# mycophonic/saprobe-alac

Measured on AMD Instinct MI355X. Metric: Msamples/s decoded (16-bit stereo, 4096-frame packets), higher is better.
Workload: dtype int32; 1 GPU; 65536 packets/GPU x 16-bit 2-ch 4096-frame ALAC, music-like synthetic, device-resident in/out; packets_per_gpu=65536

## Files before the change

saprobe-alac_amd/csrc/alac_gpu.h:

```cpp
#ifndef ALAC_GPU_H
#define ALAC_GPU_H
#include <hip/hip_runtime.h>

#include <algorithm>
#include <cstdio>
#include <cstdlib>
#include <cstring>

#define ALAC_DEV __device__ __forceinline__
#define ALAC_HD __host__ __device__ __forceinline__
#define ALAC_NOINLINE
#define ALAC_MUL24(a, b) __mul24((int)(a), (int)(b))
__device__ __forceinline__ uint32_t alac_sad(uint32_t a, uint32_t b, uint32_t c) {
    uint32_t r;
    asm("v_sad_u32 %0, %1, %2, %3" : "=v"(r) : "v"(a), "v"(b), "v"(c));
    return r;
}
#define ALAC_SAD(a, b, c) alac_sad((uint32_t)(a), (uint32_t)(b), (uint32_t)(c))

__device__ __forceinline__ int32_t alac_sign_med3(int32_t x) {
    int32_t r;
    asm("v_med3_i32 %0, %1, -1, 1" : "=v"(r) : "v"(x));
    return r;
}
#define ALAC_SIGN(x) alac_sign_med3(x)
__device__ __forceinline__ int32_t alac_clamp01_med3(int32_t x) {
    int32_t r;
    asm("v_med3_i32 %0, %1, 0, 1" : "=v"(r) : "v"(x));
    return r;
}
#define ALAC_CLAMP01(x) alac_clamp01_med3(x)
__device__ __forceinline__ uint32_t alac_xad(uint32_t a, uint32_t b, uint32_t c) {
    uint32_t r;
    asm("v_xad_u32 %0, %1, %2, %3" : "=v"(r) : "v"(a), "v"(b), "v"(c));
    return r;
}
#define ALAC_XAD(a, b, c) alac_xad((uint32_t)(a), (uint32_t)(b), (uint32_t)(c))
__device__ __forceinline__ uint32_t alac_not_add(uint32_t a, uint32_t c) {
    uint32_t r;
    asm("v_xad_u32 %0, %1, -1, %2" : "=v"(r) : "v"(a), "v"(c));
    return r;
}
#define ALAC_NOT_ADD(a, c) alac_not_add((uint32_t)(a), (uint32_t)(c))
__device__ __forceinline__ uint32_t alac_bfi(uint32_t m, uint32_t a, uint32_t b) {
    uint32_t r;
    asm("v_bfi_b32 %0, %1, %2, %3" : "=v"(r) : "v"(m), "v"(a), "v"(b));
    return r;
}
#define ALAC_BFI(m, a, b) alac_bfi((uint32_t)(m), (uint32_t)(a), (uint32_t)(b))
__device__ __forceinline__ int32_t alac_mad24(int32_t a, int32_t b, int32_t c) {
    int32_t r;
    asm("v_mad_i32_i24 %0, %1, %2, %3" : "=v"(r) : "v"(a), "v"(b), "v"(c));
    return r;
}
#define ALAC_MAD24(a, b, c) alac_mad24((int32_t)(a), (int32_t)(b), (int32_t)(c))
__device__ __forceinline__ int32_t alac_msub24(int32_t acc, int32_t a, int32_t negc) {
    int32_t r;
    asm("v_mad_i32_i24 %0, %1, %2, %3" : "=v"(r) : "v"(a), "s"(negc), "v"(acc));
    return r;
}
#define ALAC_MSUB24(acc, a, c) alac_msub24((int32_t)(acc), (int32_t)(a), -(int32_t)(c))
#define ALAC_SUBSAT(a, b) __builtin_elementwise_sub_sat((uint32_t)(a), (uint32_t)(b))
__device__ __forceinline__ uint32_t alac_ffbh(uint32_t x) {
    uint32_t r;
    asm("v_ffbh_u32 %0, %1" : "=v"(r) : "v"(x));
    return r;
}
#define ALAC_FFBH(x) alac_ffbh((uint32_t)(x))
__device__ __forceinline__ uint32_t alac_bfe(uint32_t x, uint32_t off, uint32_t width) {
    uint32_t r;
    asm("v_bfe_u32 %0, %1, %2, %3" : "=v"(r) : "v"(x), "v"(off), "v"(width));
    return r;
}
#define ALAC_BFE(x, off, width) alac_bfe((uint32_t)(x), (uint32_t)(off), (uint32_t)(width))
__device__ __forceinline__ int32_t alac_sext_bits(int32_t x, uint32_t bits) {
    int32_t r;
    asm("v_bfe_i32 %0, %1, 0, %2" : "=v"(r) : "v"(x), "v"(bits));
    return r;
}
#define ALAC_SEXT_BITS(x, bits) alac_sext_bits((int32_t)(x), (uint32_t)(bits))
#define ALAC_MULU24(a, b) __umul24((unsigned)(a), (unsigned)(b))
#define ALAC_MULHI(a, b) __umulhi((unsigned)(a), (unsigned)(b))
#define ALAC_ALIGNBIT(hi, lo, sh) __builtin_amdgcn_alignbit((unsigned)(hi), (unsigned)(lo), (unsigned)(sh))
__device__ __forceinline__ int32_t alac_med3_0(int32_t x, int32_t m) {
    int32_t r;
    asm("v_med3_i32 %0, %1, 0, %2" : "=v"(r) : "v"(x), "v"(m));
    return r;
}
#define ALAC_MED3_0(x, m) alac_med3_0((int32_t)(x), (int32_t)(m))
#define ALAC_PACK_LO16(x, y) __builtin_amdgcn_perm((uint32_t)(y), (uint32_t)(x), 0x05040100u)
#define ALAC_PACK_HI16(x, y) __builtin_amdgcn_perm((uint32_t)(y), (uint32_t)(x), 0x07060302u)
__device__ __forceinline__ uint32_t alac_pk_add16(uint32_t a, uint32_t b) {
    uint32_t r;
    asm("v_pk_add_u16 %0, %1, %2" : "=v"(r) : "v"(a), "v"(b));
    return r;
}
#define ALAC_PK_ADD16(a, b) alac_pk_add16((uint32_t)(a), (uint32_t)(b))
__device__ __forceinline__ uint32_t alac_pk_sub16(uint32_t a, uint32_t b) {
    uint32_t r;
    asm("v_pk_sub_u16 %0, %1, %2" : "=v"(r) : "v"(a), "v"(b));
    return r;
}
#define ALAC_PK_SUB16(a, b) alac_pk_sub16((uint32_t)(a), (uint32_t)(b))
#define ALAC_PICK(dst, src) asm volatile("v_mov_b32 %0, %1" : "+v"(dst) : "v"(src))
#define ALAC_OWN_REG(x) asm volatile("" : "+v"(x))
typedef uint32_t alac_u32x4_a4 __attribute__((ext_vector_type(4), aligned(4)));
#define ALAC_LOAD4(q, a, b, c, d)                                                       \
    do {                                                                                \
        const alac_u32x4_a4 v_ = *reinterpret_cast<const alac_u32x4_a4*>(q);            \
        (a) = v_.x;                                                                     \
        (b) = v_.y;                                                                     \
        (c) = v_.z;                                                                     \
        (d) = v_.w;                                                                     \
    } while (0)
typedef int32_t alac_i32x4 __attribute__((ext_vector_type(4)));
#define ALAC_LOAD4_I32(q, a, b, c, d)                                                  \
    do {                                                                               \
        const alac_i32x4 v_ = *reinterpret_cast<const alac_i32x4*>(q);  \
        (a) = v_.x;                                                                    \
        (b) = v_.y;                                                                    \
        (c) = v_.z;                                                                    \
        (d) = v_.w;                                                                    \
    } while (0)
#define ALAC_STORE4(q, a, b, c, d) (*reinterpret_cast<alac_i32x4*>(q) = alac_i32x4{(a), (b), (c), (d)})
#include "alac_wave.h"
#include "alac_regular.h"
#include "alac_duo.h"
#include "alac_split.h"

#define ALAC_PRIO_B_LONG 3
#define ALAC_PRIO_B_MID 2
#define ALAC_PRIO_B_SHORT 1
#define ALAC_PRIO_A 2
#define ALAC_PRIO_C 3

namespace alack {


typedef uint32_t u32x4 __attribute__((ext_vector_type(4)));

constexpr uint32_t kWave = 64;
constexpr uint32_t kTimingSlots = 64;
#ifndef ALAC_LDS_ROWS
#define ALAC_LDS_ROWS 64
#endif
#ifndef ALAC_LDS_RING
#define ALAC_LDS_RING 32
#endif
#ifndef ALAC_LDS_FLUSH
#define ALAC_LDS_FLUSH (ALAC_LDS_ROWS / 2)
#endif
constexpr uint32_t kRing = ALAC_LDS_ROWS;
constexpr uint32_t kFlush = ALAC_LDS_FLUSH;
static_assert(kFlush <= kRing && kRing % 4 == 0 && (kFlush == 16 || kFlush == 32), "the stager flushes 64- or 128-byte pieces of its rows");
constexpr uint32_t kRowStride = kRing + 1;
constexpr uint32_t kFallbackSlots = 64;
constexpr uint32_t kRingDw = ALAC_LDS_RING;
constexpr uint32_t kRingSlots = kRingDw + 2;

constexpr uint32_t kKeys = alac::KEY_IRREGULAR + 2u;
constexpr uint32_t kKeyLegacy = alac::KEY_IRREGULAR;
constexpr uint32_t kKeyScan = alac::KEY_IRREGULAR + 1u;
struct Plan {
    uint32_t count[kKeys];
    uint32_t pkt_start[kKeys];
    uint32_t cursor[kKeys];
    uint32_t nk;
    uint32_t list_key[kKeys];
    uint32_t list_wave0[kKeys];
    uint32_t total_waves;
    uint32_t irr_waves;
    uint32_t wide_waves;
    uint32_t gate[2][512];
    uint32_t balance[2][512];
    uint32_t queue[2];
};

static __shared__ uint32_t s_rows[kWave * kRowStride];
static __shared__ unsigned long long s_optr[kWave];
static __shared__ __attribute__((aligned(16))) uint32_t s_ring[kRingSlots * kWave];
constexpr uint32_t kQ = alac::DUO_CHUNK;
static __shared__ int32_t s_rq[2 * kQ * kWave];

__host__ __device__ inline size_t u_tile_cells(uint32_t frame_length) { return ((size_t)frame_length + 1u) * kWave; }

struct GpuWave {
    static constexpr bool kResMem = false;
    static constexpr uint32_t kRingDw = alack::kRingDw;
    int32_t* u_tile;
    int32_t* g_tile;
    uint8_t* my_out;
    uint32_t lane, wcnt, flushed;
    uint32_t ppw;

    ALAC_DEV bool any(bool p) const { return __ballot(p) != 0ull; }
    ALAC_DEV uint32_t max_u32(uint32_t v) const {
#pragma unroll
        for (int o = 32; o > 0; o >>= 1) {
            const uint32_t t = (uint32_t)__shfl_xor((int)v, o, 64);
            v = t > v ? t : v;
        }
        return (uint32_t)__builtin_amdgcn_readfirstlane((int)v);
    }
    static constexpr bool kRingPow2 = (kRing & (kRing - 1u)) == 0u;
    uint32_t wpos, fpos;
    ALAC_DEV static uint32_t umin_(uint32_t a, uint32_t b) { return a < b ? a : b; }
    ALAC_DEV static uint32_t st_wrap(uint32_t x) { return kRingPow2 ? (x & (kRing - 1u)) : umin_(x, x - kRing); }
    ALAC_DEV uint32_t st_pos() const { return kRingPow2 ? (wcnt & (kRing - 1u)) : wpos; }
    ALAC_DEV void st_adv(uint32_t n) {
        wcnt += n;
        if (!kRingPow2) wpos = st_wrap(wpos + n);
    }
    ALAC_DEV void st_begin(uint8_t* out) {
        my_out = out;
        s_optr[lane] = (unsigned long long)reinterpret_cast<uintptr_t>(out);
        wcnt = flushed = 0;
        wpos = fpos = 0;
    }
    ALAC_DEV void st_push(uint32_t v) {
        s_rows[lane * kRowStride + st_pos()] = v;
        st_adv(1u);
    }
    ALAC_DEV void st_push_if(uint32_t v, bool on) {
        s_rows[lane * kRowStride + st_pos()] = v;
        st_adv(on ? 1u : 0u);
    }
    ALAC_DEV uint32_t st_group_base(uint32_t un) const { return lane * kRowStride + (kRingPow2 ? (wcnt & (kRing - un)) : wpos); }
    ALAC_DEV void st_put(uint32_t base, uint32_t j, uint32_t v, uint32_t) { s_rows[base + j] = v; }
    ALAC_DEV void st_advance(uint32_t n) { st_adv(n); }
    ALAC_DEV void st_push6_n(uint32_t d0, uint32_t d1, uint32_t d2, uint32_t d3, uint32_t d4, uint32_t d5, uint32_t count) {
        const uint32_t pos = st_pos();
        uint32_t* row = s_rows + lane * kRowStride;
        if (pos <= kRing - 6u) {
            uint32_t* r = row + pos;
            r[0] = d0;
            r[1] = d1;
            r[2] = d2;
            r[3] = d3;
            r[4] = d4;
            r[5] = d5;
        } else {
            row[pos] = d0;
            row[st_wrap(pos + 1u)] = d1;
            row[st_wrap(pos + 2u)] = d2;
            row[st_wrap(pos + 3u)] = d3;
            row[st_wrap(pos + 4u)] = d4;
            row[st_wrap(pos + 5u)] = d5;
        }
        st_adv(count);
    }
    ALAC_DEV void st_tail(uint64_t acc, uint32_t nbytes) {
        for (uint32_t b = 0; b < nbytes; ++b) my_out[(size_t)wcnt * 4u + b] = (uint8_t)(acc >> (8u * b));
    }
    ALAC_DEV void st_step() {
        constexpr uint32_t LPP = kFlush / 4u;
        constexpr uint32_t PPI = kWave / LPP;
        const bool full = (wcnt - flushed) >= kFlush;
        const unsigned long long mask = __ballot(full);
        if (mask == 0ull) return;
        __builtin_amdgcn_wave_barrier();
        const int first = __ffsll((long long)mask) - 1;
        const uint32_t fl = (uint32_t)__shfl((int)flushed, first, 64);
        const uint32_t col0 = kRingPow2 ? (fl & (kRing - 1u)) : (uint32_t)__shfl((int)fpos, first, 64);
        const uint32_t piece = lane & (LPP - 1u);
        const uint32_t groups = (ppw + PPI - 1u) / PPI;
        const uint32_t col = st_wrap(col0 + piece * 4u);
        for (uint32_t k = 0; k < groups; ++k) {
            const uint32_t q = PPI * k + lane / LPP;
            if ((mask >> q) & 1ull) {
                const uint32_t* r = s_rows + q * kRowStride + col;
                const uint4 v = make_uint4(r[0], r[1], r[2], r[3]);
                uint8_t* dst = reinterpret_cast<uint8_t*>((uintptr_t)s_optr[q]) + ((size_t)fl + piece * 4u) * 4u;
                *reinterpret_cast<__attribute__((address_space(1))) u32x4*>((uintptr_t)dst) = u32x4{v.x, v.y, v.z, v.w};
            }
        }
        __builtin_amdgcn_wave_barrier();
        if (full) {
            flushed += kFlush;
            if (!kRingPow2) fpos = st_wrap(fpos + kFlush);
        }
    }
    ALAC_DEV uint32_t st_finish() {
        uint32_t c = kRingPow2 ? 0u : fpos;
        for (uint32_t w = flushed; w < wcnt; ++w) {
            *reinterpret_cast<uint32_t*>(my_out + (size_t)w * 4u) = s_rows[lane * kRowStride + (kRingPow2 ? (w & (kRing - 1u)) : c)];
            if (!kRingPow2) c = st_wrap(c + 1u);
        }
        flushed = wcnt;
        if (!kRingPow2) fpos = wpos;
        return wcnt;
    }
    ALAC_DEV void ring_write4(uint32_t slot, uint32_t a, uint32_t b, uint32_t c, uint32_t d) {
        uint32_t* q = &s_ring[slot * kWave + lane];
        q[0] = a;
        q[kWave] = b;
        q[2 * kWave] = c;
        q[3 * kWave] = d;
    }
    ALAC_DEV uint32_t ring_read(uint32_t slot) const { return s_ring[slot * kWave + lane]; }
    ALAC_DEV void ring_read2(uint32_t slot, uint32_t& a, uint32_t& b) const {
        const uint32_t* q = &s_ring[slot * kWave + lane];
        a = q[0];
        b = q[kWave];
    }
    ALAC_DEV void ring_read2_at(uint32_t byte_off, uint32_t& a, uint32_t& b) const {
        const uint32_t* q = reinterpret_cast<const uint32_t*>(reinterpret_cast<const char*>(&s_ring[lane]) + byte_off * kWave);
        a = q[0];
        b = q[kWave];
    }
    ALAC_DEV void ring_write1(uint32_t slot, uint32_t v) { s_ring[slot * kWave + lane] = v; }
    ALAC_DEV void rq_write(uint32_t buf, uint32_t j, int32_t v) { s_rq[(buf * kQ + j) * kWave + lane] = v; }
    ALAC_DEV int32_t rq_read(uint32_t buf, uint32_t j) const { return s_rq[(buf * kQ + j) * kWave + lane]; }
    ALAC_DEV uint32_t pair_hi(uint32_t x) const { return (uint32_t)__builtin_amdgcn_mov_dpp((int)x, 0xF5, 0xf, 0xf, true); }
    ALAC_DEV int32_t pair_sum(int32_t x) const { return x + __builtin_amdgcn_mov_dpp(x, 0xB1, 0xf, 0xf, true); }
    ALAC_DEV uint32_t pair_from_below(uint32_t x, uint32_t fresh, uint32_t q0m) const {
        return ALAC_BFI(q0m, fresh, (uint32_t)__builtin_amdgcn_mov_dpp((int)x, 0xA0, 0xf, 0xf, true));
    }
    template <int L>
    ALAC_DEV uint32_t quad_from(uint32_t x) const {
        return (uint32_t)__builtin_amdgcn_mov_dpp((int)x, L * 0x55, 0xf, 0xf, true);
    }
    template <int D>
    ALAC_DEV uint32_t quad_up(uint32_t x) const {
        constexpr int c = D == 1 ? 0xF9 : D == 2 ? 0xFE : 0xFF;
        return (uint32_t)__builtin_amdgcn_mov_dpp((int)x, c, 0xf, 0xf, true);
    }
    ALAC_DEV int32_t quad_sum(int32_t x) const {
        const int32_t y = x + __builtin_amdgcn_mov_dpp(x, 0xB1, 0xf, 0xf, true);
        return y + __builtin_amdgcn_mov_dpp(y, 0x4E, 0xf, 0xf, true);
    }
    ALAC_DEV uint32_t quad_from_below(uint32_t x, uint32_t fresh, uint32_t q0m) const {
        return ALAC_BFI(q0m, fresh, (uint32_t)__builtin_amdgcn_mov_dpp((int)x, 0x90, 0xf, 0xf, true));
    }
    ALAC_DEV void duo_sync() { asm volatile("s_waitcnt lgkmcnt(0)\n\ts_barrier" ::: "memory"); }
    ALAC_DEV void duo_sync_mem() {
        __threadfence_block();
        __syncthreads();
    }
    ALAC_DEV int32_t* u_row(uint32_t i) const { return u_tile + ((size_t)i * kWave + (ppw < kWave ? (lane < ppw ? lane : ppw) : lane)); }
    ALAC_DEV int32_t* g_slot(uint32_t k) const { return g_tile + (size_t)k * ppw; }
};

struct GpuWaveMem : GpuWave {
    static constexpr bool kResMem = true;
    const int32_t* res;
    uint32_t it, chunk0;
    ALAC_DEV int32_t rq_read(uint32_t, uint32_t j) const { return res[chunk0 + j]; }
    ALAC_DEV void rq_write(uint32_t, uint32_t, int32_t) {}
    ALAC_DEV void duo_sync() {
        ++it;
        chunk0 = (it - 1u) * kQ;
    }
    ALAC_DEV void duo_sync_mem() {}
};

__device__ __forceinline__ uint32_t avail_of(uint64_t blob_bytes, uint64_t off) {
    const uint64_t left = blob_bytes - off;
    return left > 0xffffffffull ? 0xffffffffu : (uint32_t)left;
}

__global__ void alac_classify(alac::DevCfg cfg, const uint8_t* __restrict__ blob, uint64_t blob_bytes, const uint64_t* __restrict__ offsets,
                              const uint32_t* __restrict__ sizes, uint32_t n, uint16_t* __restrict__ keys, uint32_t* __restrict__ sizes_ws,
                              uint32_t* __restrict__ frames_out, int32_t* __restrict__ status, Plan* plan);
__global__ void alac_plan(Plan* plan, uint32_t ppw);
__global__ void alac_cu_census(uint32_t* __restrict__ seen, uint32_t* __restrict__ arrived, uint32_t expect);
__global__ void alac_scatter(const uint16_t* __restrict__ keys, uint32_t n, Plan* plan, uint32_t* __restrict__ perm);
__global__ void alac_task_classify(alac::DevCfg cfg, const alac::ChanDesc* __restrict__ cd, const alac::PktDesc* __restrict__ pd,
                                   const uint16_t* __restrict__ pkt_keys, uint32_t n_slots, uint16_t* __restrict__ keys, Plan* plan);
__global__ void alac_scan(alac::DevCfg cfg, const uint8_t* __restrict__ blob, uint64_t blob_bytes, const uint64_t* __restrict__ offsets,
                          const uint32_t* __restrict__ sizes, const uint32_t* __restrict__ perm, const Plan* __restrict__ plan,
                          uint8_t* __restrict__ out, uint64_t out_stride, uint32_t* __restrict__ frames_out,
                          int32_t* __restrict__ status, int32_t* __restrict__ scratch_u, int32_t* __restrict__ scratch_g,
                          uint32_t ppw, alac::ChanDesc* __restrict__ cd, alac::PktDesc* __restrict__ pd, int32_t* __restrict__ rows,
                          uint64_t row_stride);
__global__ void alac_legacy(alac::DevCfg cfg, const uint8_t* __restrict__ blob, uint64_t blob_bytes, const uint64_t* __restrict__ offsets,
                            const uint32_t* __restrict__ sizes, const uint32_t* __restrict__ perm, const Plan* __restrict__ plan,
                            const alac::PktDesc* __restrict__ pd, uint8_t* __restrict__ out, uint64_t out_stride,
                            uint32_t* __restrict__ frames_out, int32_t* __restrict__ status, int32_t* __restrict__ scratch_u,
                            int32_t* __restrict__ scratch_g, uint32_t ppw);
constexpr uint32_t kModeFit4 = 4u, kModeFit5 = 5u, kModeGated = 6u;
constexpr __host__ __device__ __forceinline__ uint32_t decode_mode(uint32_t items, uint32_t n_cu, uint32_t cap, uint32_t force, bool mono,
                                                                  bool fit5) {
    if (force == kModeFit4 || (force == kModeFit5 && fit5)) return force;
    if (items <= 4u * n_cu) return kModeFit4;
    if (items <= 5u * n_cu) return (cap >= 5u && !mono) ? kModeGated : fit5 ? kModeFit5 : kModeFit4;
    if (items <= 6u * n_cu && cap >= 6u) return kModeGated;
    return (2u * items <= 15u * n_cu || !fit5) ? kModeFit4 : kModeFit5;
}
constexpr __host__ __device__ __forceinline__ uint32_t pair_quota(uint32_t items, uint32_t n_cu, uint32_t cap) {
    const uint32_t need = (items + n_cu - 1u) / n_cu;
    return need < 5u ? 5u : need < cap ? need : cap;
}
constexpr bool mode_is_fit4_without_the_others(uint32_t n_cu) {
    for (uint32_t items = 0u; items <= 40u * n_cu; items += (items < 8u * n_cu ? 1u : n_cu / 2u + 1u))
        if (decode_mode(items, n_cu, 0u, 0u, false, false) != kModeFit4 || decode_mode(items, n_cu, 0u, 5u, true, false) != kModeFit4) return false;
    return true;
}
constexpr bool mode_is_fit4_within_four(uint32_t n_cu) {
    for (uint32_t cap = 0u; cap <= 8u; ++cap)
        for (uint32_t items = 0u; items <= 4u * n_cu; ++items)
            if (decode_mode(items, n_cu, cap, 0u, false, true) != kModeFit4 || decode_mode(items, n_cu, cap, 0u, true, true) != kModeFit4) return false;
    return true;
}
static_assert(mode_is_fit4_without_the_others(1u) && mode_is_fit4_without_the_others(64u) && mode_is_fit4_without_the_others(256u) &&
                  mode_is_fit4_within_four(1u) && mode_is_fit4_within_four(7u) && mode_is_fit4_within_four(64u) &&
                  mode_is_fit4_within_four(256u) && mode_is_fit4_within_four(304u),
              "decode_mode would leave batches of up to 4 x CUs wave slots to a launch that is not made for them");
constexpr uint32_t kQuadLdsFit4 = 34816u;

struct PairArgs {
    alac::DevCfg cfg;
    const uint8_t* blob;
    uint64_t blob_bytes;
    const uint64_t* offsets;
    const uint32_t* sizes;
    const uint32_t* perm;
    Plan* plan;
    uint8_t* out;
    uint64_t out_stride;
    uint32_t* frames_out;
    int32_t* status;
    int32_t* scratch_u;
    const uint32_t* cu_number;
    uint32_t* claims;
    uint32_t ppw;
    uint32_t n_cu;
    uint32_t cap;
    uint32_t lanes_min;
    uint32_t fit;
    uint32_t fit_force;
    uint32_t fit5;
};
#define ALAC_DECLARE_DECODE(NAME) __global__ void NAME(PairArgs);
ALAC_DECLARE_DECODE(alac_decode_16q) ALAC_DECLARE_DECODE(alac_decode_16g) ALAC_DECLARE_DECODE(alac_decode_24q) ALAC_DECLARE_DECODE(alac_decode_32q)
ALAC_DECLARE_DECODE(alac_decode_w24) ALAC_DECLARE_DECODE(alac_decode_w32)
#undef ALAC_DECLARE_DECODE
__global__ void alac_chan_predict(alac::DevCfg cfg, const uint8_t* __restrict__ blob, uint64_t blob_bytes, const uint64_t* __restrict__ offsets,
                                  const uint32_t* __restrict__ sizes, const uint32_t* __restrict__ perm, const Plan* __restrict__ plan,
                                  const alac::ChanDesc* __restrict__ cd, int32_t* __restrict__ rows, uint64_t row_stride, uint32_t ppw);
__global__ void alac_interleave(alac::DevCfg cfg, const uint8_t* __restrict__ blob, uint64_t blob_bytes, const uint64_t* __restrict__ offsets,
                                const uint32_t* __restrict__ sizes, const uint32_t* __restrict__ perm, const Plan* __restrict__ plan,
                                const alac::ChanDesc* __restrict__ cd, const alac::PktDesc* __restrict__ pd, const int32_t* __restrict__ rows,
                                uint64_t row_stride, uint8_t* __restrict__ out, uint64_t out_stride, uint32_t blocks_per_pkt);
__global__ void alac_interleave4(alac::DevCfg cfg, const uint8_t* __restrict__ blob, uint64_t blob_bytes, const uint64_t* __restrict__ offsets,
                                const uint32_t* __restrict__ sizes, const uint32_t* __restrict__ perm, const Plan* __restrict__ plan,
                                const alac::ChanDesc* __restrict__ cd, const alac::PktDesc* __restrict__ pd, const int32_t* __restrict__ rows,
                                uint64_t row_stride, uint8_t* __restrict__ out, uint64_t out_stride, uint32_t blocks_per_pkt);

}
#endif
```

saprobe-alac_amd/csrc/alacgpu.hip:

```cpp
#include "alac_gpu.h"
#include "alac_host.h"
#include "alac_waveform.h"
#include "alac_clips.h"

using namespace alack;

namespace {
thread_local char g_err[512] = "";
}

void alack::set_err(const char* fmt, ...) {
    va_list ap;
    va_start(ap, fmt);
    vsnprintf(g_err, sizeof(g_err), fmt, ap);
    va_end(ap);
}

namespace {

class CopyPool {
public:
    explicit CopyPool(unsigned threads) {
        for (unsigned t = 0; t < threads; ++t) workers_.emplace_back([this] { run(); });
    }
    ~CopyPool() {
        {
            std::lock_guard<std::mutex> g(m_);
            stop_ = true;
        }
        cv_.notify_all();
        for (auto& w : workers_) w.join();
    }
    void parallel_for(size_t tasks, const std::function<void(size_t)>& fn) {
        if (tasks == 0) return;
        if (workers_.empty() || tasks == 1) {
            for (size_t k = 0; k < tasks; ++k) fn(k);
            return;
        }
        {
            std::lock_guard<std::mutex> g(m_);
            fn_ = &fn;
            tasks_ = tasks;
            next_ = 0;
            left_ = tasks;
            ++gen_;
        }
        cv_.notify_all();
        work();
        std::unique_lock<std::mutex> l(m_);
        done_.wait(l, [this] { return left_ == 0; });
        fn_ = nullptr;
    }

private:
    void work() {
        for (;;) {
            size_t k;
            const std::function<void(size_t)>* fn;
            {
                std::lock_guard<std::mutex> g(m_);
                if (!fn_ || next_ >= tasks_) return;
                k = next_++;
                fn = fn_;
            }
            (*fn)(k);
            std::lock_guard<std::mutex> g(m_);
            if (--left_ == 0) done_.notify_all();
        }
    }
    void run() {
        uint64_t seen = 0;
        for (;;) {
            {
                std::unique_lock<std::mutex> l(m_);
                cv_.wait(l, [&] { return stop_ || gen_ != seen; });
                if (stop_) return;
                seen = gen_;
            }
            work();
        }
    }
    std::vector<std::thread> workers_;
    std::mutex m_;
    std::condition_variable cv_, done_;
    const std::function<void(size_t)>* fn_ = nullptr;
    size_t tasks_ = 0, next_ = 0, left_ = 0;
    uint64_t gen_ = 0;
    bool stop_ = false;
};

void copy_pieces(CopyPool* pool, size_t pieces, const std::function<void(size_t)>& fn) {
    if (pool) pool->parallel_for(pieces, fn);
    else for (size_t k = 0; k < pieces; k++) fn(k);
}

constexpr int kSlots = 3;

struct Slot {
    DevBuf d_in;
    DevBuf d_out;
    HostBuf h_in, h_out;
    hipEvent_t ev_in = nullptr, ev_k = nullptr, ev_out = nullptr;
    size_t first = 0, n = 0;
    bool busy = false;
    bool bad = false;
};

struct PairKernel {
    void (*fn)(PairArgs);
    const char* name;
};
struct Kernels {
    bool lean;
    bool one_or_two;
    PairKernel quad;
    PairKernel gated;
    PairKernel wide;
    decltype(&alac_interleave) interleave;
    uint32_t interleave_lds;
    const char* irregular;
};
#define ALAC_PAIR_KERNEL(k) PairKernel{k, #k}
Kernels choose_kernels(const alac::DevCfg& c) {
    Kernels k{};
    k.lean = alac::lean_config(c);
    k.one_or_two = c.num_channels <= 2;
    k.quad = c.bit_depth == 16 ? ALAC_PAIR_KERNEL(alac_decode_16q) : c.bit_depth == 32 ? ALAC_PAIR_KERNEL(alac_decode_32q) : ALAC_PAIR_KERNEL(alac_decode_24q);
    k.gated = c.bit_depth == 16 ? ALAC_PAIR_KERNEL(alac_decode_16g) : PairKernel{nullptr, ""};
    k.wide = c.bit_depth == 32 ? ALAC_PAIR_KERNEL(alac_decode_w32) : c.bit_depth == 24 ? ALAC_PAIR_KERNEL(alac_decode_w24) : PairKernel{nullptr, ""};
    const bool four_frames = c.num_channels > 2 && (c.num_channels * c.bps) % 4u == 0u;
    k.interleave = four_frames ? alac_interleave4 : alac_interleave;
    k.interleave_lds = (four_frames ? 128u : 32u) * kWave;
    k.irregular = !k.lean        ? "alac_scan (whole-packet decoder)"
                  : k.one_or_two ? "alac_scan + alac_interleave (+ alac_legacy)"
                  : four_frames  ? "alac_scan + alac_chan_predict + alac_interleave4 (+ alac_legacy)"
                                 : "alac_scan + alac_chan_predict + alac_interleave (+ alac_legacy)";
    return k;
}
#undef ALAC_PAIR_KERNEL

}

struct alacgpu_decoder {
    alacgpu_config cfg;
    alac::DevCfg dev_cfg;
    Kernels kernels;
    int device;
    size_t frame_bytes;
    hipStream_t stream;
    hipStream_t s_in, s_out;
    hipStream_t s_side;
    hipEvent_t ev_fork, ev_join;
    hipEvent_t ev_start[kTimingSlots], ev_stop[kTimingSlots];
    uint64_t launches;
    DevBuf scratch_u, scratch_g, plan, cls, perm, sizes_ws;
    DevBuf cd, pd, plan2, keys2, perm2, rows;
    Slot slots[kSlots];
    CopyPool* pool;
    uint32_t n_cu;
    DevBuf cu_number;
    size_t chunk_bytes;
    uint32_t lanes_min;
    int side;
    std::thread* ahead;
    int ahead_rc;
    char ahead_err[512];
    size_t last_n;
    uint32_t last_ppw, last_cap, last_fit5;
    uint32_t fit_force;
    DevBuf wave_ws;
    hipEvent_t ev_w0, ev_w1;
    bool wave_timed;
    hipEvent_t ev_c0, ev_c1;
    bool clips_timed;
};

namespace {

size_t plan_claims_offset() { return (sizeof(Plan) + 255u) & ~(size_t)255u; }
size_t plan_bytes(size_t waves) { return plan_claims_offset() + waves * 4 * sizeof(uint32_t); }

struct KernelAttr {
    uint32_t pairs_per_cu, static_lds;
};
KernelAttr kernel_attr(void (*kernel)(PairArgs)) {
    static std::mutex mu;
    static std::vector<std::pair<const void*, KernelAttr>> cache;
    std::lock_guard<std::mutex> g(mu);
    for (const auto& e : cache)
        if (e.first == (const void*)kernel) return e.second;
    int v = 0;
    hipFuncAttributes at;
    KernelAttr a{4u, kQuadLdsFit4};
    if (hipOccupancyMaxActiveBlocksPerMultiprocessor(&v, kernel, (int)(2 * kWave), 0) == hipSuccess && v > 0) a.pairs_per_cu = (uint32_t)v;
    else (void)hipGetLastError();
    if (hipFuncGetAttributes(&at, (const void*)kernel) == hipSuccess) a.static_lds = (uint32_t)at.sharedSizeBytes;
    else (void)hipGetLastError();
    cache.emplace_back((const void*)kernel, a);
    return a;
}

int cu_numbers(alacgpu_decoder* dec) {
    int rc;
    if ((rc = dec->cu_number.ensure(513 * sizeof(uint32_t)))) return rc;
    HIP_TRY(hipMemsetAsync(dec->cu_number.p, 0, 513 * sizeof(uint32_t), dec->stream));
    hipLaunchKernelGGL(alac_cu_census, dim3(2 * dec->n_cu), dim3(kWave), 0, dec->stream, (uint32_t*)dec->cu_number.p,
                       (uint32_t*)dec->cu_number.p + 512, 2 * dec->n_cu);
    HIP_TRY(hipGetLastError());
    uint32_t seen[512];
    HIP_TRY(hipMemcpyAsync(seen, dec->cu_number.p, sizeof(seen), hipMemcpyDeviceToHost, dec->stream));
    HIP_TRY(hipStreamSynchronize(dec->stream));
    uint32_t per_xcd[8] = {0}, xcds = 0, total = 0;
    for (uint32_t i = 0; i < 512; i++)
        if (seen[i]) {
            per_xcd[i >> 6]++;
            total++;
        }
    for (uint32_t x = 0; x < 8; x++) xcds += per_xcd[x] ? 1u : 0u;
    if (xcds == 0) xcds = 1;
    uint32_t next[8] = {0}, order[8] = {0}, k = 0;
    for (uint32_t x = 0; x < 8; x++)
        if (per_xcd[x]) order[x] = k++;
    for (uint32_t i = 0; i < 512; i++)
        if (seen[i]) {
            const uint32_t x = i >> 6;
            seen[i] = 1u + next[x]++ * xcds + order[x];
        }
    if (total > dec->n_cu) dec->n_cu = total;
    HIP_TRY(hipMemcpyAsync(dec->cu_number.p, seen, sizeof(seen), hipMemcpyHostToDevice, dec->stream));
    HIP_TRY(hipStreamSynchronize(dec->stream));
    return ALACGPU_E_OK;
}

size_t max_waves(uint32_t bit_depth, size_t n, uint32_t ppw) {
    const size_t keys = (bit_depth >= 24 ? 2 : 1) * 18 * 18 + 8;
    return (n + ppw - 1) / ppw + std::min<size_t>(n, keys);
}
size_t max_waves(const alacgpu_decoder* dec, size_t n, uint32_t ppw) { return max_waves(dec->cfg.bit_depth, n, ppw); }

uint32_t pick_ppw(size_t n) {
    if (const char* e = getenv("ALACGPU_PPW")) {
        const int v = atoi(e);
        if (v >= 1 && v <= 64) return (uint32_t)v;
    }
    uint32_t ppw = kWave;
    while (ppw > 1 && n / ppw < 256) ppw >>= 1;
    return ppw;
}

size_t row_stride_of(uint32_t frame_length) { return ((size_t)frame_length + 3u) & ~(size_t)3u; }

int reserve_workspace(alacgpu_decoder* dec, size_t n, uint32_t ppw) {
    const size_t waves = max_waves(dec, n, ppw);
    int rc;
    if ((rc = dec->scratch_u.ensure(waves * u_tile_cells(dec->cfg.frame_length) * sizeof(int32_t)))) return rc;
    if ((rc = dec->scratch_g.ensure(waves * kFallbackSlots * ppw * sizeof(int32_t)))) return rc;
    if ((rc = dec->plan.ensure(plan_bytes(waves)))) return rc;
    if ((rc = dec->cls.ensure((n ? n : 1) * sizeof(uint16_t)))) return rc;
    if ((rc = dec->perm.ensure((n ? n : 1) * sizeof(uint32_t)))) return rc;
    if ((rc = dec->sizes_ws.ensure((n ? n : 1) * sizeof(uint32_t)))) return rc;
    const size_t ns = (n ? n : 1) * 8;
    if ((rc = dec->cd.ensure(ns * sizeof(alac::ChanDesc)))) return rc;
    if ((rc = dec->pd.ensure((n ? n : 1) * sizeof(alac::PktDesc)))) return rc;
    if (dec->cfg.num_channels > 2) {
        if ((rc = dec->plan2.ensure(sizeof(Plan)))) return rc;
        if ((rc = dec->keys2.ensure(ns * sizeof(uint16_t)))) return rc;
        if ((rc = dec->perm2.ensure(ns * sizeof(uint32_t)))) return rc;
        if ((rc = dec->rows.ensure((n ? n : 1) * dec->cfg.num_channels * row_stride_of(dec->cfg.frame_length) * sizeof(int32_t))))
            return rc;
    }
    return ALACGPU_E_OK;
}

struct Launch {
    alacgpu_decoder* dec;
    alac::DevCfg c;
    const uint8_t* d_blob;
    uint64_t blob_bytes;
    const uint64_t* d_offsets;
    size_t n;
    uint8_t* d_out;
    size_t out_stride;
    uint32_t* d_frames;
    int32_t* d_status;
    uint32_t ppw;
    size_t waves;
    hipStream_t irr;
    bool forked;
    uint32_t scan_grid;
    Plan* plan() const { return (Plan*)dec->plan.p; }
    const uint32_t* sz() const { return (const uint32_t*)dec->sizes_ws.p; }
};

struct SideFork {
    alacgpu_decoder* dec;
    bool open = false;
    int fork() {
        HIP_TRY(hipEventRecord(dec->ev_fork, dec->stream));
        HIP_TRY(hipStreamWaitEvent(dec->s_side, dec->ev_fork, 0));
        open = true;
        return ALACGPU_E_OK;
    }
    int join() {
        HIP_TRY(hipEventRecord(dec->ev_join, dec->s_side));
        HIP_TRY(hipStreamWaitEvent(dec->stream, dec->ev_join, 0));
        open = false;
        return ALACGPU_E_OK;
    }
    ~SideFork() {
        if (open) (void)hipStreamSynchronize(dec->s_side);
    }
};

int sort_pass(const Launch& L, const uint32_t* d_sizes) {
    alacgpu_decoder* dec = L.dec;
    const uint32_t nb = (uint32_t)((L.n + 255) / 256);
    HIP_TRY(hipMemsetAsync(L.plan(), 0, plan_bytes(L.waves), dec->stream));
    hipLaunchKernelGGL(alac_classify, dim3(nb), dim3(256), 0, dec->stream, L.c, L.d_blob, L.blob_bytes, L.d_offsets, d_sizes,
                       (uint32_t)L.n, (uint16_t*)dec->cls.p, (uint32_t*)dec->sizes_ws.p, L.d_frames, L.d_status, L.plan());
    hipLaunchKernelGGL(alac_plan, dim3(1), dim3(kWave), 0, dec->stream, L.plan(), L.ppw);
    hipLaunchKernelGGL(alac_scatter, dim3(nb), dim3(256), 0, dec->stream, (const uint16_t*)dec->cls.p, (uint32_t)L.n, L.plan(),
                       (uint32_t*)dec->perm.p);
    return ALACGPU_E_OK;
}

void scan(const Launch& L) {
    alacgpu_decoder* dec = L.dec;
    hipLaunchKernelGGL(alac_scan, dim3(L.scan_grid), dim3(kWave), 0, L.irr, L.c, L.d_blob, L.blob_bytes,
                       L.d_offsets, L.sz(), (const uint32_t*)dec->perm.p, (const Plan*)L.plan(), L.d_out, (uint64_t)L.out_stride, L.d_frames,
                       L.d_status, (int32_t*)dec->scratch_u.p, (int32_t*)dec->scratch_g.p, L.ppw, (alac::ChanDesc*)dec->cd.p,
                       (alac::PktDesc*)dec->pd.p, dec->cfg.num_channels > 2 ? (int32_t*)dec->rows.p : (int32_t*)nullptr,
                       (uint64_t)row_stride_of(dec->cfg.frame_length));
}

void narrow_launch(const Launch& L, const PairArgs& a, uint32_t slots, uint32_t mode) {
    alacgpu_decoder* dec = L.dec;
    const Kernels& k = dec->kernels;
    if (mode == kModeGated) {
        if (a.cap) hipLaunchKernelGGL(k.gated.fn, dim3(std::min<uint32_t>(a.cap * dec->n_cu, slots)), dim3(2 * kWave), 0, dec->stream, a);
        return;
    }
    if (mode == kModeFit5 && !a.fit5) return;
    const uint32_t stat = kernel_attr(k.quad.fn).static_lds;
    PairArgs q = a;
    q.fit = mode;
    hipLaunchKernelGGL(k.quad.fn, dim3(slots), dim3(4 * kWave), (mode == kModeFit4 && stat < kQuadLdsFit4) ? kQuadLdsFit4 - stat : 0u,
                       dec->stream, q);
}

void regular_packets(const Launch& L) {
    alacgpu_decoder* dec = L.dec;
    const Kernels& k = dec->kernels;
    const size_t n = L.n;
    const uint32_t ppw = L.ppw;
    PairArgs a{L.c, L.d_blob, (uint64_t)L.blob_bytes, L.d_offsets, L.sz(), (const uint32_t*)dec->perm.p, L.plan(), L.d_out, (uint64_t)L.out_stride,
               L.d_frames, L.d_status, (int32_t*)dec->scratch_u.p, (const uint32_t*)dec->cu_number.p,
               (uint32_t*)((uint8_t*)L.plan() + plan_claims_offset()), ppw, dec->n_cu, 0u, dec->lanes_min, 4u, dec->fit_force, 0u};
    const uint32_t slots = (uint32_t)L.waves;
    const uint32_t n_cu = dec->n_cu;
    const bool beyond4 = (n + ppw - 1) / ppw > (size_t)4 * n_cu || dec->fit_force == kModeFit5;
    const bool has_twin = k.gated.fn && beyond4 && dec->fit_force == 0u;
    {
        const uint32_t stat = kernel_attr(k.quad.fn).static_lds;
        a.fit5 = (beyond4 && (size_t)((stat + 1279u) / 1280u) * 1280u * 5u <= 163840u) ? 1u : 0u;
    }
    if (has_twin) a.cap = kernel_attr(k.gated.fn).pairs_per_cu;
    if (a.cap <= 4u) a.cap = 0u;
    dec->last_cap = a.cap;
    dec->last_fit5 = a.fit5;
    const uint32_t guess = decode_mode((uint32_t)((n + ppw - 1) / ppw), n_cu, a.cap, dec->fit_force, dec->cfg.num_channels == 1, a.fit5 != 0u);
    narrow_launch(L, a, slots, guess);
    if (k.wide.fn) hipLaunchKernelGGL(k.wide.fn, dim3(slots), dim3(2 * kWave), 0, dec->stream, a);
    for (uint32_t mode : {kModeFit4, kModeFit5, kModeGated})
        if (mode != guess) narrow_launch(L, a, slots, mode);
}

int split_pipeline(const Launch& L) {
    alacgpu_decoder* dec = L.dec;
    Plan* plan2 = (Plan*)dec->plan2.p;
    const size_t n_slots = L.n * 8;
    const uint32_t nb2 = (uint32_t)((n_slots + 255) / 256);
    const uint32_t ppw2 = pick_ppw(L.n * dec->cfg.num_channels);
    HIP_TRY(hipMemsetAsync(plan2, 0, sizeof(Plan), dec->stream));
    hipLaunchKernelGGL(alac_task_classify, dim3(nb2), dim3(256), 0, dec->stream, L.c, (const alac::ChanDesc*)dec->cd.p,
                       (const alac::PktDesc*)dec->pd.p, (const uint16_t*)dec->cls.p, (uint32_t)n_slots,
                       (uint16_t*)dec->keys2.p, plan2);
    hipLaunchKernelGGL(alac_plan, dim3(1), dim3(kWave), 0, dec->stream, plan2, ppw2);
    hipLaunchKernelGGL(alac_scatter, dim3(nb2), dim3(256), 0, dec->stream, (const uint16_t*)dec->keys2.p,
                       (uint32_t)n_slots, plan2, (uint32_t*)dec->perm2.p);
    hipLaunchKernelGGL(alac_chan_predict, dim3((uint32_t)max_waves(16u, n_slots, ppw2)), dim3(kWave), 0, dec->stream, L.c,
                       L.d_blob, L.blob_bytes, L.d_offsets, L.sz(), (const uint32_t*)dec->perm2.p, (const Plan*)plan2,
                       (const alac::ChanDesc*)dec->cd.p, (int32_t*)dec->rows.p, (uint64_t)row_stride_of(dec->cfg.frame_length), ppw2);
    return ALACGPU_E_OK;
}

void irregular_pcm(const Launch& L) {
    alacgpu_decoder* dec = L.dec;
    const Kernels& k = dec->kernels;
    const uint64_t rs = row_stride_of(dec->cfg.frame_length);
    const uint32_t bpp = (dec->cfg.frame_length + kWave - 1u) / kWave;
    const uint32_t ib = (uint32_t)std::min<uint64_t>((uint64_t)L.n * ((bpp + 7u) / 8u), L.forked ? (uint64_t)4 * dec->n_cu : (uint64_t)32768u);
    hipLaunchKernelGGL(k.interleave, dim3(ib), dim3(kWave), k.interleave_lds, L.irr, L.c, L.d_blob, L.blob_bytes, L.d_offsets, L.sz(),
                       (const uint32_t*)dec->perm.p, (const Plan*)L.plan(), (const alac::ChanDesc*)dec->cd.p,
                       (const alac::PktDesc*)dec->pd.p, (const int32_t*)dec->rows.p, rs, L.d_out, (uint64_t)L.out_stride, bpp);
    hipLaunchKernelGGL(alac_legacy, dim3(L.scan_grid), dim3(kWave), 0, L.irr, L.c, L.d_blob, L.blob_bytes,
                       L.d_offsets, L.sz(), (const uint32_t*)dec->perm.p, (const Plan*)L.plan(), (const alac::PktDesc*)dec->pd.p, L.d_out,
                       (uint64_t)L.out_stride, L.d_frames, L.d_status, (int32_t*)dec->scratch_u.p, (int32_t*)dec->scratch_g.p, L.ppw);
}

int launch(alacgpu_decoder* dec, const uint8_t* d_blob, uint64_t blob_bytes, const uint64_t* d_offsets,
           const uint32_t* d_sizes, size_t n, uint8_t* d_out, size_t out_stride, uint32_t* d_frames, int32_t* d_status) {
    if (n == 0) return ALACGPU_E_OK;
    if (n > 0x7fffffffu) {
        set_err("batch too large");
        return ALACGPU_E_ARG;
    }
    const uint32_t ppw = pick_ppw(n);
    int rc = reserve_workspace(dec, n, ppw);
    if (rc) return rc;
    dec->last_n = n;
    dec->last_ppw = ppw;
    dec->last_cap = dec->last_fit5 = 0;
    const Kernels& k = dec->kernels;
    Launch L{dec, dec->dev_cfg, d_blob, blob_bytes, d_offsets, n, d_out, out_stride, d_frames, d_status, ppw, max_waves(dec, n, ppw),
             dec->stream, false, 0u};
    L.c.aligned16 = (out_stride % 16 == 0 && (reinterpret_cast<uintptr_t>(d_out) % 16) == 0) ? 1u : 0u;
    const uint32_t slot = (uint32_t)(dec->launches % kTimingSlots);
    HIP_TRY(hipEventRecord(dec->ev_start[slot], dec->stream));
    if ((rc = sort_pass(L, d_sizes))) return rc;
    L.forked = k.one_or_two && k.lean &&
               (dec->side >= 2 || (dec->side == 1 && (n + ppw - 1) / ppw <= (size_t)6 * dec->n_cu));
    L.scan_grid = (uint32_t)std::min<size_t>(L.waves, (size_t)(L.forked ? 2u : 6u) * dec->n_cu);
    SideFork side{dec};
    if (L.forked) {
        if ((rc = side.fork())) return rc;
        L.irr = dec->s_side;
    }
    if (!L.forked) scan(L);
    if (k.one_or_two && k.lean) regular_packets(L);
    if (L.forked) scan(L);
    HIP_TRY(hipGetLastError());
    if (k.lean) {
        if (!k.one_or_two && (rc = split_pipeline(L))) return rc;
        irregular_pcm(L);
        HIP_TRY(hipGetLastError());
    }
    if (L.forked && (rc = side.join())) return rc;
    HIP_TRY(hipEventRecord(dec->ev_stop[slot], dec->stream));
    dec->launches++;
    return ALACGPU_E_OK;
}

}

namespace {
std::mutex g_pool_mu;
std::vector<alacgpu_decoder*> g_pool;
std::vector<std::pair<void*, size_t>> g_host_pool;
std::vector<std::pair<void*, size_t>> g_host_sizes;
constexpr size_t kPoolPerDevice = 4;
constexpr size_t kPoolKeepDevice = (size_t)2048 << 20;
constexpr size_t kPoolKeepPinned = (size_t)64 << 20;
constexpr size_t kHostPoolBlock = (size_t)64 << 20, kHostPoolBytes = (size_t)192 << 20, kHostPoolCount = 8;
template <class Buf>
void keep_at_most(std::vector<Buf*> bufs, size_t limit) {
    for (;;) {
        size_t total = 0;
        Buf* big = nullptr;
        for (Buf* b : bufs) {
            total += b->cap;
            if (b->cap && (!big || b->cap > big->cap)) big = b;
        }
        if (total <= limit || !big) return;
        big->release();
    }
}

std::vector<DevBuf*> device_buffers(alacgpu_decoder* d) {
    std::vector<DevBuf*> v = {&d->scratch_u, &d->scratch_g, &d->plan, &d->cls, &d->perm, &d->sizes_ws, &d->cd, &d->pd,
                              &d->plan2, &d->keys2, &d->perm2, &d->rows, &d->wave_ws};
    for (Slot& s : d->slots) v.insert(v.end(), {&s.d_in, &s.d_out});
    return v;
}
std::vector<HostBuf*> pinned_buffers(alacgpu_decoder* d) {
    std::vector<HostBuf*> v;
    for (Slot& s : d->slots) v.insert(v.end(), {&s.h_in, &s.h_out});
    return v;
}
std::vector<hipStream_t*> streams_of(alacgpu_decoder* d) { return {&d->stream, &d->s_in, &d->s_out, &d->s_side}; }
struct EventRef {
    hipEvent_t* ev;
    unsigned flags;
};
std::vector<EventRef> events_of(alacgpu_decoder* d) {
    std::vector<EventRef> v = {{&d->ev_fork, hipEventDisableTiming}, {&d->ev_join, hipEventDisableTiming},
                               {&d->ev_w0, hipEventDefault}, {&d->ev_w1, hipEventDefault},
                               {&d->ev_c0, hipEventDefault}, {&d->ev_c1, hipEventDefault}};
    for (uint32_t i = 0; i < kTimingSlots; i++) v.insert(v.end(), {{&d->ev_start[i], hipEventDefault}, {&d->ev_stop[i], hipEventDefault}});
    for (Slot& s : d->slots)
        v.insert(v.end(), {{&s.ev_in, hipEventDisableTiming}, {&s.ev_k, hipEventDisableTiming}, {&s.ev_out, hipEventDisableTiming}});
    return v;
}

bool synchronize_all(alacgpu_decoder* d) {
    bool ok = true;
    for (hipStream_t* s : streams_of(d))
        if (*s && hipStreamSynchronize(*s) != hipSuccess) ok = false;
    return ok;
}

void really_destroy(alacgpu_decoder* d) {
    (void)hipSetDevice(d->device);
    (void)synchronize_all(d);
    delete d->pool;
    d->cu_number.release();
    for (DevBuf* b : device_buffers(d)) b->release();
    for (HostBuf* b : pinned_buffers(d)) b->release();
    for (const EventRef& e : events_of(d))
        if (*e.ev) (void)hipEventDestroy(*e.ev);
    for (hipStream_t* s : streams_of(d))
        if (*s) (void)hipStreamDestroy(*s);
    delete d;
}

void configure(alacgpu_decoder* d, const alacgpu_config* cfg) {
    const uint32_t bps = alacwf::bytes_per_sample(cfg->bit_depth);
    d->cfg = *cfg;
    d->frame_bytes = (size_t)cfg->frame_length * cfg->num_channels * (size_t)bps;
    d->dev_cfg = alac::DevCfg{cfg->frame_length, cfg->bit_depth, cfg->num_channels, cfg->pb, cfg->mb, cfg->kb, bps, 0u};
    d->kernels = choose_kernels(d->dev_cfg);
    d->launches = 0;
    d->ahead = nullptr;
    d->ahead_rc = ALACGPU_E_OK;
    d->ahead_err[0] = 0;
    d->last_n = 0;
    d->last_ppw = d->last_cap = d->last_fit5 = 0;
    d->wave_timed = false;
    d->clips_timed = false;
    d->lanes_min = 4;
    d->fit_force = 0;
    if (const char* e = getenv("ALACGPU_FIT")) d->fit_force = (uint32_t)atoi(e);
    if (const char* e = getenv("ALACGPU_LANES_MIN")) d->lanes_min = (uint32_t)std::max(1, atoi(e));
    d->side = 2;
    if (const char* e = getenv("ALACGPU_SIDE")) d->side = atoi(e);
    d->chunk_bytes = (size_t)192 << 20;
    if (const char* e = getenv("ALACGPU_CHUNK_MB")) {
        const long v = atol(e);
        if (v >= 1 && v <= 65536) d->chunk_bytes = (size_t)v << 20;
    }
}
}

static int settle_ahead(alacgpu_decoder* d);

static int check_decode_args(const alacgpu_decoder* d, const void* blob, size_t blob_bytes, const void* offsets, size_t n, const void* out,
                             size_t out_stride, const void* frames, const void* status) {
    if (!d || (n && (!offsets || !out || !frames || !status)) || (blob_bytes && !blob)) {
        set_err("null argument");
        return ALACGPU_E_ARG;
    }
    if (out_stride < d->frame_bytes) {
        set_err("out_stride %zu < frame bytes %zu", out_stride, d->frame_bytes);
        return ALACGPU_E_ARG;
    }
    return ALACGPU_E_OK;
}

extern "C" {

int alacgpu_create(const alacgpu_config* cfg, int device, alacgpu_decoder** out) {
    if (!cfg || !out) {
        set_err("null argument");
        return ALACGPU_E_ARG;
    }
    *out = nullptr;
    if (int rc = check_config(cfg)) return rc;
    HIP_TRY(hipSetDevice(device));
    {
        std::lock_guard<std::mutex> g(g_pool_mu);
        for (size_t i = 0; i < g_pool.size(); i++)
            if (g_pool[i]->device == device) {
                alacgpu_decoder* d = g_pool[i];
                g_pool.erase(g_pool.begin() + (long)i);
                configure(d, cfg);
                *out = d;
                return ALACGPU_E_OK;
            }
    }
    alacgpu_decoder* d = new (std::nothrow) alacgpu_decoder();
    if (!d) {
        set_err("out of memory");
        return ALACGPU_E_ARG;
    }
    d->device = device;
    configure(d, cfg);
    {
        int cus = 0;
        if (hipDeviceGetAttribute(&cus, hipDeviceAttributeMultiprocessorCount, device) != hipSuccess) cus = 0;
        d->n_cu = cus > 0 ? (uint32_t)cus : 256u;
    }
    hipError_t e = hipSuccess;
    for (hipStream_t* st : streams_of(d))
        if (e == hipSuccess) e = hipStreamCreateWithFlags(st, hipStreamNonBlocking);
    for (const EventRef& ev : events_of(d))
        if (e == hipSuccess) e = hipEventCreateWithFlags(ev.ev, ev.flags);
    if (e != hipSuccess) {
        set_err("stream/event creation failed: %s", hipGetErrorString(e));
        really_destroy(d);
        return ALACGPU_E_HIP;
    }
    if (int rc = cu_numbers(d)) {
        really_destroy(d);
        return rc;
    }
    *out = d;
    return ALACGPU_E_OK;
}

void alacgpu_destroy(alacgpu_decoder* d) {
    if (!d) return;
    (void)settle_ahead(d);
    (void)hipSetDevice(d->device);
    if (synchronize_all(d)) {
        for (int k = 0; k < kSlots; k++) d->slots[k].busy = false;
        keep_at_most(device_buffers(d), kPoolKeepDevice);
        keep_at_most(pinned_buffers(d), kPoolKeepPinned);
        std::lock_guard<std::mutex> g(g_pool_mu);
        size_t same = 0;
        for (alacgpu_decoder* p : g_pool) same += p->device == d->device ? 1u : 0u;
        if (same < kPoolPerDevice) {
            g_pool.push_back(d);
            return;
        }
    }
    really_destroy(d);
}

void alacgpu_trim(void) {
    std::vector<alacgpu_decoder*> all;
    std::vector<std::pair<void*, size_t>> host;
    {
        std::lock_guard<std::mutex> g(g_pool_mu);
        all.swap(g_pool);
        host.swap(g_host_pool);
    }
    for (alacgpu_decoder* d : all) really_destroy(d);
    for (auto& h : host) (void)hipHostFree(h.first);
}

void* alacgpu_host_alloc(size_t bytes) {
    if (bytes == 0) bytes = 1;
    {
        std::lock_guard<std::mutex> g(g_pool_mu);
        size_t best = SIZE_MAX;
        for (size_t i = 0; i < g_host_pool.size(); i++)
            if (g_host_pool[i].second >= bytes && g_host_pool[i].second <= 2 * bytes + (1u << 20) &&
                (best == SIZE_MAX || g_host_pool[i].second < g_host_pool[best].second))
                best = i;
        if (best != SIZE_MAX) {
            void* p = g_host_pool[best].first;
            g_host_sizes.emplace_back(p, g_host_pool[best].second);
            g_host_pool.erase(g_host_pool.begin() + (long)best);
            return p;
        }
    }
    void* p = nullptr;
    if (hipHostMalloc(&p, bytes, hipHostMallocDefault) != hipSuccess) {
        (void)hipGetLastError();
        set_err("hipHostMalloc(%zu) failed", bytes);
        return nullptr;
    }
    std::lock_guard<std::mutex> g(g_pool_mu);
    g_host_sizes.emplace_back(p, bytes);
    return p;
}

void alacgpu_host_free(void* p) {
    if (!p) return;
    size_t bytes = 0;
    std::vector<void*> evict;
    {
        std::lock_guard<std::mutex> g(g_pool_mu);
        for (size_t i = 0; i < g_host_sizes.size(); i++)
            if (g_host_sizes[i].first == p) {
                bytes = g_host_sizes[i].second;
                g_host_sizes.erase(g_host_sizes.begin() + (long)i);
                break;
            }
        if (bytes && bytes <= kHostPoolBlock) {
            g_host_pool.emplace_back(p, bytes);
            p = nullptr;
            size_t total = 0;
            for (const auto& h : g_host_pool) total += h.second;
            while (g_host_pool.size() > kHostPoolCount || total > kHostPoolBytes) {
                evict.push_back(g_host_pool.front().first);
                total -= g_host_pool.front().second;
                g_host_pool.erase(g_host_pool.begin());
            }
        }
    }
    for (void* q : evict) (void)hipHostFree(q);
    if (p) (void)hipHostFree(p);
}

int alacgpu_get_format(const alacgpu_decoder* d, alacgpu_format* fmt) {
    if (!d || !fmt) return ALACGPU_E_ARG;
    fmt->sample_rate = (int32_t)d->cfg.sample_rate;
    fmt->bit_depth = d->cfg.bit_depth;
    fmt->channels = d->cfg.num_channels;
    return ALACGPU_E_OK;
}

size_t alacgpu_frame_bytes(const alacgpu_decoder* d) { return d ? d->frame_bytes : 0; }

int alacgpu_reserve(alacgpu_decoder* d, size_t n) {
    if (!d) return ALACGPU_E_ARG;
    HIP_TRY(hipSetDevice(d->device));
    if (int rc = d->wave_ws.ensure(alack::wave_scratch_bytes(n))) return rc;
    return reserve_workspace(d, n, pick_ppw(n));
}

static int settle_ahead(alacgpu_decoder* d) {
    if (!d->ahead) return ALACGPU_E_OK;
    d->ahead->join();
    delete d->ahead;
    d->ahead = nullptr;
    if (d->ahead_rc != ALACGPU_E_OK) set_err("%s", d->ahead_err);
    return d->ahead_rc;
}

int alacgpu_decode_batch_start(alacgpu_decoder* d, const uint8_t* blob, size_t blob_bytes, const uint64_t* offsets, size_t n,
                               uint8_t* out, size_t out_stride, uint32_t* frames_out, int32_t* status) {
    if (!d) return ALACGPU_E_ARG;
    if (d->ahead) {
        set_err("a decode started with alacgpu_decode_batch_start is still in flight: alacgpu_decode_batch_wait first");
        return ALACGPU_E_ARG;
    }
    d->ahead_rc = ALACGPU_E_OK;
    d->ahead = new (std::nothrow) std::thread([=] {
        d->ahead_rc = alacgpu_decode_batch(d, blob, blob_bytes, offsets, n, out, out_stride, frames_out, status);
        if (d->ahead_rc != ALACGPU_E_OK) snprintf(d->ahead_err, sizeof(d->ahead_err), "%s", alacgpu_last_error());
    });
    if (!d->ahead) {
        set_err("out of memory");
        return ALACGPU_E_ARG;
    }
    return ALACGPU_E_OK;
}

int alacgpu_decode_batch_wait(alacgpu_decoder* d) {
    if (!d) return ALACGPU_E_ARG;
    return settle_ahead(d);
}

int alacgpu_decode_batch_device(alacgpu_decoder* d, const uint8_t* d_blob, size_t blob_bytes, const uint64_t* d_offsets,
                                const uint32_t* d_sizes, size_t n, uint8_t* d_out, size_t out_stride,
                                uint32_t* d_frames, int32_t* d_status, int sync) {
    int rc = check_decode_args(d, d_blob, blob_bytes, d_offsets, n, d_out, out_stride, d_frames, d_status);
    if (rc) return rc;
    HIP_TRY(hipSetDevice(d->device));
    rc = launch(d, d_blob, (uint64_t)blob_bytes, d_offsets, d_sizes, n, d_out, out_stride, d_frames, d_status);
    if (rc) return rc;
    if (sync) HIP_TRY(hipStreamSynchronize(d->stream));
    return ALACGPU_E_OK;
}

int alacgpu_decode_batch(alacgpu_decoder* d, const uint8_t* blob, size_t blob_bytes, const uint64_t* offsets, size_t n,
                         uint8_t* out, size_t out_stride, uint32_t* frames_out, int32_t* status) {
    if (int rc = check_decode_args(d, blob, blob_bytes, offsets, n, out, out_stride, frames_out, status)) return rc;
    if (n == 0) return ALACGPU_E_OK;
    auto valid = [&](size_t i) {
        const uint64_t lo = offsets[i], hi = offsets[i + 1];
        return lo <= hi && hi <= (uint64_t)blob_bytes && hi - lo <= 0x0fffffffull;
    };
    HIP_TRY(hipSetDevice(d->device));
    const size_t fb = d->frame_bytes;
    const size_t d_stride = (fb + 15u) & ~(size_t)15u;
    const bool out_pinned = is_pinned(out) && is_pinned(frames_out) && is_pinned(status);
    const bool in_pinned = blob_bytes == 0 || is_pinned(blob);
    if (!d->pool && !(out_pinned && in_pinned)) {
        unsigned t = std::thread::hardware_concurrency();
        t = t > 16 ? 8 : (t > 2 ? t / 2 : 1);
        if (const char* e = getenv("ALACGPU_COPY_THREADS")) t = (unsigned)std::max(1, atoi(e));
        d->pool = new (std::nothrow) CopyPool(t - 1);
    }

    auto finish = [&](Slot& s) -> int {
        HIP_TRY(hipEventSynchronize(s.ev_out));
        if (!out_pinned) {
            const uint8_t* h = (const uint8_t*)s.h_out.p;
            const uint8_t* hm = h + s.n * d_stride;
            memcpy(frames_out + s.first, hm, s.n * sizeof(uint32_t));
            memcpy(status + s.first, hm + s.n * sizeof(uint32_t), s.n * sizeof(int32_t));
            const size_t pieces = std::min<size_t>(s.n, 64);
            auto body = [&](size_t k) {
                const size_t lo = s.n * k / pieces, hi = s.n * (k + 1) / pieces;
                if (out_stride == fb && d_stride == fb) {
                    memcpy(out + (s.first + lo) * out_stride, h + lo * d_stride, (hi - lo) * fb);
                } else {
                    for (size_t i = lo; i < hi; i++) memcpy(out + (s.first + i) * out_stride, h + i * d_stride, fb);
                }
            };
            copy_pieces(d->pool, pieces, body);
        }
        if (s.bad)
            for (size_t i = s.first; i < s.first + s.n; i++)
                if (!valid(i)) {
                    status[i] = ALACGPU_ERR_RANGE;
                    frames_out[i] = 0;
                }
        {
            const size_t bpf = fb / d->cfg.frame_length;
            for (size_t i = s.first; i < s.first + s.n; i++) {
                const size_t have = std::min<size_t>(frames_out[i], d->cfg.frame_length) * bpf;
                if (have < fb) memset(out + i * out_stride + have, 0, fb - have);
            }
        }
        s.busy = false;
        return ALACGPU_E_OK;
    };
    auto submit = [&](Slot& s, size_t first, size_t cnt, uint64_t lo, uint64_t hi) -> int {
        int rc;
        s.first = first;
        s.n = cnt;
        s.bad = false;
        const size_t in_bytes = (size_t)(hi - lo);
        const size_t meta = (cnt + 1) * sizeof(uint64_t) + cnt * sizeof(uint32_t);
        const size_t meta_pad = (meta + 255u) & ~(size_t)255u;
        if ((rc = s.d_in.ensure(meta_pad + in_bytes + 16))) return rc;
        if ((rc = s.d_out.ensure(cnt * d_stride + cnt * 8 + 16))) return rc;
        if ((rc = s.h_in.ensure(in_pinned ? meta_pad : meta_pad + in_bytes))) return rc;
        if (!out_pinned && (rc = s.h_out.ensure(cnt * d_stride + cnt * 8))) return rc;
        uint64_t* h_off = (uint64_t*)s.h_in.p;
        uint32_t* h_sz = (uint32_t*)(h_off + cnt + 1);
        for (size_t i = 0; i < cnt; i++) {
            const bool ok = valid(first + i);
            h_off[i] = ok ? offsets[first + i] - lo : 0u;
            h_sz[i] = ok ? (uint32_t)(offsets[first + i + 1] - offsets[first + i]) : 0u;
            s.bad = s.bad || !ok;
        }
        h_off[cnt] = in_bytes;
        uint8_t* d_in = (uint8_t*)s.d_in.p;
        if (in_pinned) {
            HIP_TRY(hipMemcpyAsync(d_in, h_off, meta, hipMemcpyHostToDevice, d->s_in));
            if (in_bytes) HIP_TRY(hipMemcpyAsync(d_in + meta_pad, blob + lo, in_bytes, hipMemcpyHostToDevice, d->s_in));
        } else {
            uint8_t* hb = (uint8_t*)s.h_in.p + meta_pad;
            const size_t pieces = std::max<size_t>(1, std::min<size_t>(64, in_bytes >> 20));
            auto body = [&](size_t k) {
                const size_t a = in_bytes * k / pieces, b = in_bytes * (k + 1) / pieces;
                memcpy(hb + a, blob + lo + a, b - a);
            };
            copy_pieces(d->pool, pieces, body);
            HIP_TRY(hipMemcpyAsync(d_in, s.h_in.p, meta_pad + in_bytes, hipMemcpyHostToDevice, d->s_in));
        }
        HIP_TRY(hipEventRecord(s.ev_in, d->s_in));
        HIP_TRY(hipStreamWaitEvent(d->stream, s.ev_in, 0));
        uint8_t* d_pcm = (uint8_t*)s.d_out.p;
        uint32_t* d_fr = (uint32_t*)(d_pcm + cnt * d_stride);
        int32_t* d_st = (int32_t*)(d_fr + cnt);
        if ((rc = launch(d, d_in + meta_pad, in_bytes, (const uint64_t*)d_in, (const uint32_t*)(d_in + (cnt + 1) * sizeof(uint64_t)), cnt,
                         d_pcm, d_stride, d_fr, d_st)))
            return rc;
        HIP_TRY(hipEventRecord(s.ev_k, d->stream));
        HIP_TRY(hipStreamWaitEvent(d->s_out, s.ev_k, 0));
        if (out_pinned) {
            HIP_TRY(hipMemcpy2DAsync(out + first * out_stride, out_stride, d_pcm, d_stride, fb, cnt, hipMemcpyDeviceToHost, d->s_out));
            HIP_TRY(hipMemcpyAsync(frames_out + first, d_fr, cnt * sizeof(uint32_t), hipMemcpyDeviceToHost, d->s_out));
            HIP_TRY(hipMemcpyAsync(status + first, d_st, cnt * sizeof(int32_t), hipMemcpyDeviceToHost, d->s_out));
        } else {
            HIP_TRY(hipMemcpyAsync(s.h_out.p, d_pcm, cnt * d_stride + cnt * 8, hipMemcpyDeviceToHost, d->s_out));
        }
        HIP_TRY(hipEventRecord(s.ev_out, d->s_out));
        s.busy = true;
        return ALACGPU_E_OK;
    };

    size_t first = 0;
    int turn = 0;
    int rc = ALACGPU_E_OK;
    while (first < n && rc == ALACGPU_E_OK) {
        size_t cnt = 0;
        uint64_t lo = ~0ull, hi = 0;
        while (first + cnt < n) {
            uint64_t nlo = lo, nhi = hi;
            if (valid(first + cnt)) {
                nlo = std::min(lo, offsets[first + cnt]);
                nhi = std::max(hi, offsets[first + cnt + 1]);
            }
            const uint64_t bytes = (nhi > nlo ? nhi - nlo : 0) + (uint64_t)(cnt + 1) * fb;
            if (cnt != 0 && bytes > d->chunk_bytes) break;
            lo = nlo;
            hi = nhi;
            cnt++;
        }
        if (hi < lo) lo = hi = 0;
        Slot& s = d->slots[turn];
        turn = (turn + 1) % kSlots;
        if (s.busy && (rc = finish(s))) break;
        rc = submit(s, first, cnt, lo, hi);
        first += cnt;
    }
    if (rc != ALACGPU_E_OK) {
        (void)hipStreamSynchronize(d->s_in);
        (void)hipStreamSynchronize(d->stream);
        (void)hipStreamSynchronize(d->s_side);
        (void)hipStreamSynchronize(d->s_out);
        for (int k = 0; k < kSlots; k++) d->slots[k].busy = false;
        return rc;
    }
    for (int k = 0; k < kSlots; k++) {
        Slot& s = d->slots[(turn + k) % kSlots];
        if (!s.busy) continue;
        const int r2 = finish(s);
        if (rc == ALACGPU_E_OK) rc = r2;
        s.busy = false;
    }
    return rc;
}

int alacgpu_decode_packet(alacgpu_decoder* d, const uint8_t* packet, size_t packet_len, uint8_t* out, size_t out_cap,
                          size_t* out_len, int32_t* status_out) {
    if (!d || (!packet && packet_len) || !out || !out_len) {
        set_err("null argument");
        return ALACGPU_E_ARG;
    }
    if (out_cap < d->frame_bytes) {
        set_err("output capacity %zu < frame bytes %zu", out_cap, d->frame_bytes);
        return ALACGPU_E_ARG;
    }
    *out_len = 0;
    const uint64_t offs[2] = {0, packet_len};
    const uint8_t dummy = 0;
    uint32_t frames = 0;
    int32_t st = 0;
    int rc = alacgpu_decode_batch(d, packet_len ? packet : &dummy, packet_len, offs, 1, out, d->frame_bytes, &frames, &st);
    if (rc) return rc;
    if (status_out) *status_out = st;
    if (st != 0) {
        set_err("decode failed: status 0x%x", st);
        return ALACGPU_E_DECODE;
    }
    *out_len = (size_t)frames * d->cfg.num_channels * (size_t)d->dev_cfg.bps;
    return ALACGPU_E_OK;
}

int alacgpu_timing_reset(alacgpu_decoder* d) {
    if (!d) return ALACGPU_E_ARG;
    d->launches = 0;
    return ALACGPU_E_OK;
}

int alacgpu_kernel_times(alacgpu_decoder* d, float* ms, size_t max_n, size_t* n_out) {
    if (!d || !ms || !n_out) return ALACGPU_E_ARG;
    HIP_TRY(hipSetDevice(d->device));
    HIP_TRY(hipStreamSynchronize(d->stream));
    size_t avail = (size_t)std::min<uint64_t>(d->launches, kTimingSlots);
    size_t n = std::min(avail, max_n);
    for (size_t i = 0; i < n; i++) {
        const uint32_t slot = (uint32_t)((d->launches - n + i) % kTimingSlots);
        HIP_TRY(hipEventElapsedTime(&ms[i], d->ev_start[slot], d->ev_stop[slot]));
    }
    *n_out = n;
    return ALACGPU_E_OK;
}

int alacgpu_pair_placement(alacgpu_decoder* d, uint32_t* tags, size_t max_n, size_t* n_out) {
    if (!d || !tags || !n_out) return ALACGPU_E_ARG;
    HIP_TRY(hipSetDevice(d->device));
    HIP_TRY(hipStreamSynchronize(d->stream));
    *n_out = 0;
    if (!d->plan.p) return ALACGPU_E_OK;
    Plan head;
    HIP_TRY(hipMemcpy(&head, d->plan.p, sizeof(Plan), hipMemcpyDeviceToHost));
    const size_t n = std::min<size_t>(head.total_waves, max_n / 4);
    if (plan_bytes(n) > d->plan.cap) return ALACGPU_E_ARG;
    if (n) HIP_TRY(hipMemcpy(tags, (const uint8_t*)d->plan.p + plan_claims_offset(), n * 4 * sizeof(uint32_t), hipMemcpyDeviceToHost));
    *n_out = n;
    return ALACGPU_E_OK;
}

int alacgpu_last_dispatch(alacgpu_decoder* d, alacgpu_dispatch* out) {
    if (!d || !out) return ALACGPU_E_ARG;
    HIP_TRY(hipSetDevice(d->device));
    HIP_TRY(hipStreamSynchronize(d->stream));
    memset(out, 0, sizeof(*out));
    if (!d->plan.p || d->last_n == 0) return ALACGPU_E_OK;
    Plan head;
    HIP_TRY(hipMemcpy(&head, d->plan.p, sizeof(Plan), hipMemcpyDeviceToHost));
    out->packets_per_slot = d->last_ppw;
    out->slots = head.total_waves;
    out->irregular_slots = head.irr_waves;
    out->wide_slots = head.wide_waves;
    out->narrow_slots = head.total_waves - head.irr_waves - head.wide_waves;
    out->keys = head.nk;
    const Kernels& k = d->kernels;
    const bool lean = k.one_or_two && k.lean;
    const char* narrow = "";
    if (lean && out->narrow_slots) {
        const uint32_t mode = decode_mode(out->narrow_slots, d->n_cu, d->last_cap, d->fit_force, d->cfg.num_channels == 1, d->last_fit5 != 0u);
        narrow = mode == kModeGated ? k.gated.name : k.quad.name;
        out->gated = mode == kModeGated ? 1u : 0u;
        out->workgroups_per_cu = mode == kModeGated ? pair_quota(out->narrow_slots, d->n_cu, d->last_cap) : mode;
        if (!out->gated && out->narrow_slots <= d->n_cu + d->n_cu / 8u && d->lanes_min <= 16u) out->lanes_per_packet = d->last_ppw <= 32u ? 4u : 2u;
    }
    snprintf(out->narrow_kernel, sizeof(out->narrow_kernel), "%s", narrow);
    snprintf(out->wide_kernel, sizeof(out->wide_kernel), "%s", (lean && out->wide_slots) ? k.wide.name : "");
    snprintf(out->irregular_kernels, sizeof(out->irregular_kernels), "%s", out->irregular_slots ? k.irregular : "");
    return ALACGPU_E_OK;
}

int alacgpu_last_kernel_ms(alacgpu_decoder* d, float* ms) {
    size_t got = 0;
    int rc = alacgpu_kernel_times(d, ms, 1, &got);
    if (rc) return rc;
    if (got == 0) {
        set_err("no kernel has been launched on this handle since the last timing reset");
        return ALACGPU_E_ARG;
    }
    return ALACGPU_E_OK;
}

int alacgpu_waveform_device(alacgpu_decoder* d, const uint8_t* d_pcm, size_t pcm_stride, const uint32_t* d_frames,
                            const int32_t* d_status, size_t n, int layout, int type, void* d_wave, size_t channel_stride,
                            size_t packet_stride, uint64_t* d_starts, int sync) {
    if (!d || (n && (!d_pcm || !d_frames || !d_wave))) {
        set_err("null argument");
        return ALACGPU_E_ARG;
    }
    if ((layout != ALACGPU_WAVE_STREAM && layout != ALACGPU_WAVE_PACKETS) || (type != ALACGPU_WAVE_FLOAT && type != ALACGPU_WAVE_INT)) {
        set_err("unknown waveform layout %d or type %d", layout, type);
        return ALACGPU_E_ARG;
    }
    if (n > 0x7fffffffu) {
        set_err("batch too large");
        return ALACGPU_E_ARG;
    }
    const uint64_t fl = d->cfg.frame_length, ch = d->cfg.num_channels;
    if (n) {
        if (pcm_stride < d->frame_bytes) {
            set_err("pcm_stride %zu < frame bytes %zu", pcm_stride, d->frame_bytes);
            return ALACGPU_E_ARG;
        }
        if (reinterpret_cast<uintptr_t>(d_wave) % 4) {
            set_err("d_wave is not aligned to its 4-byte elements");
            return ALACGPU_E_ARG;
        }
        if (layout == ALACGPU_WAVE_STREAM ? channel_stride < (uint64_t)n * fl
                                          : (channel_stride < fl || packet_stride / ch < channel_stride)) {
            set_err("channel_stride %zu / packet_stride %zu too small for %zu packets of %u frames", channel_stride, packet_stride, n,
                    d->cfg.frame_length);
            return ALACGPU_E_ARG;
        }
    }
    HIP_TRY(hipSetDevice(d->device));
    if (n && (layout == ALACGPU_WAVE_STREAM || d_starts)) {
        if (int rc = d->wave_ws.ensure(alack::wave_scratch_bytes(n))) return rc;
    }
    alacwf::Params p = alacwf::make_params(d->cfg.frame_length, d->cfg.bit_depth, d->cfg.num_channels, (uint32_t)layout, (uint32_t)type);
    p.pcm = d_pcm;
    p.pcm_stride = pcm_stride;
    p.frames = d_frames;
    p.status = d_status;
    p.wave = (uint8_t*)d_wave;
    p.channel_stride = channel_stride;
    p.packet_stride = packet_stride;
    p.n = n;
    HIP_TRY(hipEventRecord(d->ev_w0, d->stream));
    HIP_TRY(alack::wave_launch(d->stream, p, d_starts, d->wave_ws.p));
    HIP_TRY(hipEventRecord(d->ev_w1, d->stream));
    d->wave_timed = true;
    if (sync) HIP_TRY(hipStreamSynchronize(d->stream));
    return ALACGPU_E_OK;
}

int alacgpu_waveform_last_ms(alacgpu_decoder* d, float* ms) {
    if (!d || !ms || !d->wave_timed) {
        set_err(!d || !ms ? "null argument" : "no waveform pass on this handle yet");
        return ALACGPU_E_ARG;
    }
    HIP_TRY(hipSetDevice(d->device));
    HIP_TRY(hipEventSynchronize(d->ev_w1));
    HIP_TRY(hipEventElapsedTime(ms, d->ev_w0, d->ev_w1));
    return ALACGPU_E_OK;
}

int alacgpu_clips_device(alacgpu_decoder* d, const uint8_t* d_pcm, size_t pcm_stride, const uint32_t* d_frames,
                         const int32_t* d_status, size_t n, const uint64_t* d_begin, const uint64_t* d_limit, size_t n_clips,
                         uint32_t clip_frames, int type, void* d_clips, size_t channel_stride, size_t clip_stride,
                         uint32_t* d_valid, int32_t* d_clip_status, int sync) {
    if (!d || (n_clips && (!d_pcm || !d_frames || !d_begin || !d_limit || !d_clips))) {
        set_err("null argument");
        return ALACGPU_E_ARG;
    }
    if (type != ALACGPU_WAVE_FLOAT && type != ALACGPU_WAVE_INT) {
        set_err("unknown waveform type %d", type);
        return ALACGPU_E_ARG;
    }
    if (n > 0x7fffffffu || n_clips > 0x7fffffffu) {
        set_err("batch too large");
        return ALACGPU_E_ARG;
    }
    if (n_clips == 0) return ALACGPU_E_OK;
    const uint64_t ch = d->cfg.num_channels;
    if (clip_frames == 0) {
        set_err("clip_frames is 0");
        return ALACGPU_E_ARG;
    }
    if (n && (pcm_stride < d->frame_bytes || pcm_stride > SIZE_MAX / n)) {
        set_err("pcm_stride %zu < frame bytes %zu, or the slots overflow", pcm_stride, d->frame_bytes);
        return ALACGPU_E_ARG;
    }
    if (reinterpret_cast<uintptr_t>(d_clips) % 4) {
        set_err("d_clips is not aligned to its 4-byte elements");
        return ALACGPU_E_ARG;
    }
    if (channel_stride < clip_frames || clip_stride / ch < channel_stride || clip_stride > (SIZE_MAX / 8) / n_clips) {
        set_err("channel_stride %zu / clip_stride %zu too small for clips of %u frames, or the clips overflow", channel_stride, clip_stride,
                clip_frames);
        return ALACGPU_E_ARG;
    }
    HIP_TRY(hipSetDevice(d->device));
    alacclip::Params p = alacclip::make_params(d->cfg.frame_length, d->cfg.bit_depth, d->cfg.num_channels, (uint32_t)type, clip_frames);
    p.pcm = d_pcm;
    p.pcm_stride = pcm_stride;
    p.frames = d_frames;
    p.status = d_status;
    p.n = n;
    p.begin = d_begin;
    p.limit = d_limit;
    p.n_clips = n_clips;
    p.clips = (uint8_t*)d_clips;
    p.channel_stride = channel_stride;
    p.clip_stride = clip_stride;
    p.valid = d_valid;
    p.clip_status = d_clip_status;
    HIP_TRY(hipEventRecord(d->ev_c0, d->stream));
    HIP_TRY(alack::clips_launch(d->stream, p));
    HIP_TRY(hipEventRecord(d->ev_c1, d->stream));
    d->clips_timed = true;
    if (sync) HIP_TRY(hipStreamSynchronize(d->stream));
    return ALACGPU_E_OK;
}

int alacgpu_clips_last_ms(alacgpu_decoder* d, float* ms) {
    if (!d || !ms || !d->clips_timed) {
        set_err(!d || !ms ? "null argument" : "no clip gather on this handle yet");
        return ALACGPU_E_ARG;
    }
    HIP_TRY(hipSetDevice(d->device));
    HIP_TRY(hipEventSynchronize(d->ev_c1));
    HIP_TRY(hipEventElapsedTime(ms, d->ev_c0, d->ev_c1));
    return ALACGPU_E_OK;
}

void* alacgpu_stream(alacgpu_decoder* d) { return d ? (void*)d->stream : nullptr; }

int alacgpu_synchronize(alacgpu_decoder* d) {
    if (!d) return ALACGPU_E_ARG;
    HIP_TRY(hipSetDevice(d->device));
    HIP_TRY(hipStreamSynchronize(d->stream));
    return ALACGPU_E_OK;
}

const char* alacgpu_last_error(void) { return g_err; }

const char* alacgpu_version(void) { return "alacgpu 0.7.0 gfx950"; }

}
```

saprobe-alac_amd/csrc/k_sort.hip:

```cpp
#include "alac_gpu.h"

namespace alack {

__global__ void __launch_bounds__(256)
alac_classify(alac::DevCfg cfg, const uint8_t* __restrict__ blob, uint64_t blob_bytes, const uint64_t* __restrict__ offsets,
              const uint32_t* __restrict__ sizes, uint32_t n, uint16_t* __restrict__ keys, uint32_t* __restrict__ sizes_ws,
              uint32_t* __restrict__ frames_out, int32_t* __restrict__ status, Plan* plan) {
    __shared__ uint32_t hist[kKeys];
    for (uint32_t k = threadIdx.x; k < kKeys; k += blockDim.x) hist[k] = 0;
    __syncthreads();
    const uint32_t i = blockIdx.x * blockDim.x + threadIdx.x;
    if (i < n) {
        const uint64_t off = offsets[i];
        uint64_t sz = sizes ? (uint64_t)sizes[i] : offsets[i + 1] - off;
        const bool ok = off <= blob_bytes && sz <= blob_bytes - off && sz <= 0x0fffffffull &&
                        (sizes || offsets[i + 1] >= off);
        if (!ok) {
            keys[i] = (uint16_t)alac::TASK_NONE;
            sizes_ws[i] = 0;
            frames_out[i] = 0;
            status[i] = ALACGPU_ERR_RANGE;
        } else if (sz == 0) {
            keys[i] = (uint16_t)alac::TASK_NONE;
            sizes_ws[i] = 0;
            frames_out[i] = 0;
            status[i] = ALACGPU_STATUS(alac::ST_OVERRUN, 0, 0);
        } else {
            sizes_ws[i] = (uint32_t)sz;
            const uint8_t* p = blob + off;
            uint32_t key = alac::classify_regular(cfg, p, (uint32_t)sz, avail_of(blob_bytes, off));
            if (key == alac::KEY_IRREGULAR) key = alac::lean_config(cfg) ? kKeyScan : kKeyLegacy;
            keys[i] = (uint16_t)key;
            atomicAdd(&hist[key], 1u);
        }
    }
    __syncthreads();
    for (uint32_t k = threadIdx.x; k < kKeys; k += blockDim.x)
        if (hist[k]) atomicAdd(&plan->count[k], hist[k]);
}

__global__ void __launch_bounds__(kWave) alac_plan(Plan* plan, uint32_t ppw) {
    __shared__ uint32_t cnt[kKeys];
    for (uint32_t k = threadIdx.x; k < kKeys; k += kWave) cnt[k] = plan->count[k];
    __syncthreads();
    constexpr uint32_t R = (kKeys + kWave - 1) / kWave;
    const uint32_t q0 = threadIdx.x * R;
    uint32_t p = 0, w = 0, z = 0, wi = 0, ww = 0;
    for (uint32_t r = 0; r < R; ++r) {
        const uint32_t q = q0 + r;
        if (q >= kKeys) break;
        const uint32_t key = kKeys - 1u - q;
        const uint32_t c = cnt[key];
        const uint32_t cw = (c + ppw - 1) / ppw;
        p += c;
        w += cw;
        z += c ? 1u : 0u;
        wi += key >= alac::KEY_IRREGULAR ? cw : 0u;
        ww += (key >= alac::KEY_WIDE && key < alac::KEY_IRREGULAR) ? cw : 0u;
    }
    uint32_t ip = p, iw = w, iz = z, ii = wi, ix = ww;
#pragma unroll
    for (int o = 1; o < (int)kWave; o <<= 1) {
        const uint32_t tp = (uint32_t)__shfl_up((int)ip, o, kWave), tw = (uint32_t)__shfl_up((int)iw, o, kWave);
        const uint32_t tz = (uint32_t)__shfl_up((int)iz, o, kWave), ti = (uint32_t)__shfl_up((int)ii, o, kWave);
        const uint32_t tx = (uint32_t)__shfl_up((int)ix, o, kWave);
        if ((int)threadIdx.x >= o) {
            ix += tx;
            ip += tp;
            iw += tw;
            iz += tz;
            ii += ti;
        }
    }
    uint32_t ep = ip - p, ew = iw - w, ez = iz - z;
    for (uint32_t r = 0; r < R; ++r) {
        const uint32_t q = q0 + r;
        if (q >= kKeys) break;
        const uint32_t key = kKeys - 1u - q;
        const uint32_t c = cnt[key];
        plan->pkt_start[key] = ep;
        plan->cursor[key] = 0;
        if (c) {
            plan->list_key[ez] = key;
            plan->list_wave0[ez] = ew;
            ++ez;
            ep += c;
            ew += (c + ppw - 1) / ppw;
        }
    }
    if (threadIdx.x == kWave - 1u) {
        plan->nk = iz;
        plan->total_waves = iw;
        plan->irr_waves = ii;
        plan->wide_waves = ix;
    }
}

__global__ void __launch_bounds__(256)
alac_scatter(const uint16_t* __restrict__ keys, uint32_t n, Plan* plan, uint32_t* __restrict__ perm) {
    __shared__ uint32_t hist[kKeys];
    __shared__ uint32_t base[kKeys];
    for (uint32_t k = threadIdx.x; k < kKeys; k += blockDim.x) hist[k] = 0;
    __syncthreads();
    const uint32_t i = blockIdx.x * blockDim.x + threadIdx.x;
    uint32_t key = 0, local = 0;
    if (i < n) {
        key = keys[i];
        if (key != alac::TASK_NONE) local = atomicAdd(&hist[key], 1u);
    }
    __syncthreads();
    for (uint32_t k = threadIdx.x; k < kKeys; k += blockDim.x)
        if (hist[k]) base[k] = plan->pkt_start[k] + atomicAdd(&plan->cursor[k], hist[k]);
    __syncthreads();
    if (i < n && key != alac::TASK_NONE) perm[base[key] + local] = i;
}

__global__ void __launch_bounds__(256)
alac_task_classify(alac::DevCfg cfg, const alac::ChanDesc* __restrict__ cd, const alac::PktDesc* __restrict__ pd,
                   const uint16_t* __restrict__ pkt_keys, uint32_t n_slots, uint16_t* __restrict__ keys, Plan* plan) {
    __shared__ uint32_t hist[alac::NUM_TASK_KEYS];
    if (threadIdx.x < alac::NUM_TASK_KEYS) hist[threadIdx.x] = 0;
    __syncthreads();
    const uint32_t t = blockIdx.x * blockDim.x + threadIdx.x;
    if (t < n_slots) {
        const uint32_t pkt = t >> 3, slot = t & 7u;
        uint32_t key = alac::TASK_NONE;
        if (pkt_keys[pkt] == kKeyScan) {
            const alac::PktDesc q = pd[pkt];
            if (q.status == 0 && q.route == alac::ROUTE_SPLIT && slot < q.nslots) {
                const alac::ChanDesc d = cd[t];
                if ((d.info & alac::CD_VALID) && !(d.info & alac::CD_ESCAPE)) key = alac::chan_task_key(cfg, d);
            }
        }
        keys[t] = (uint16_t)key;
        if (key != alac::TASK_NONE) atomicAdd(&hist[key], 1u);
    }
    __syncthreads();
    if (threadIdx.x < alac::NUM_TASK_KEYS && hist[threadIdx.x]) atomicAdd(&plan->count[threadIdx.x], hist[threadIdx.x]);
}

__global__ void __launch_bounds__(kWave) alac_cu_census(uint32_t* __restrict__ seen, uint32_t* __restrict__ arrived, uint32_t expect) {
    __shared__ uint32_t pad[16384];
    pad[threadIdx.x] = threadIdx.x;
    if (threadIdx.x == 0) {
        uint32_t id, xcc;
        asm volatile("s_getreg_b32 %0, hwreg(HW_REG_HW_ID)" : "=s"(id));
        asm volatile("s_getreg_b32 %0, hwreg(HW_REG_XCC_ID)" : "=s"(xcc));
        seen[((xcc & 7u) << 6) | (((id >> 13) & 3u) << 4) | ((id >> 8) & 15u)] = 1u;
        atomicAdd(arrived, 1u);
        for (int i = 0; i < 4000 && atomicAdd(arrived, 0u) < expect; ++i) __builtin_amdgcn_s_sleep(32);
    }
    __syncthreads();
    if (pad[(threadIdx.x * 5u) & 63u] == 0xffffffffu) seen[0] = 2u;
}

}
```

Baseline: 260,100 Msamples/s.

## Fold plan kernel into classify, double-buffer plans, run classify ahead on side stream

Removes the separate single-block alac_plan launch: the last block of classify/task_classify, picked with a ticket counter, computes the plan scan. The per-launch plan memsets are gone too. Plans are double-buffered and the other half is wiped inside the scatter kernel, and the status/frames writes for invalid packets move into scatter. Classify can run on a separate pre-pass stream gated by the previous launch's scatter event, so it may overlap the tail of the previous decode. This adds stream and event management and a last-block fence pattern, plus error-recovery logic that re-zeroes plans after an aborted launch.

```diff
diff --git a/saprobe-alac_amd/csrc/alac_gpu.h b/saprobe-alac_amd/csrc/alac_gpu.h
--- a/saprobe-alac_amd/csrc/alac_gpu.h
+++ b/saprobe-alac_amd/csrc/alac_gpu.h
@@ -161,6 +161,9 @@
 constexpr uint32_t kKeys = alac::KEY_IRREGULAR + 2u;
 constexpr uint32_t kKeyLegacy = alac::KEY_IRREGULAR;
 constexpr uint32_t kKeyScan = alac::KEY_IRREGULAR + 1u;
+constexpr uint32_t kKeyEmpty = alac::TASK_NONE;
+constexpr uint32_t kKeyRange = alac::TASK_NONE - 1u;
+static_assert(kKeyRange >= kKeys && kKeyEmpty == 0xffffu, "the verdict keys lie above every sort key and fit 16 bits");
 struct Plan {
     uint32_t count[kKeys];
     uint32_t pkt_start[kKeys];
@@ -174,6 +177,7 @@
     uint32_t gate[2][512];
     uint32_t balance[2][512];
     uint32_t queue[2];
+    uint32_t ticket;
 };
 
 static __shared__ uint32_t s_rows[kWave * kRowStride];
@@ -361,12 +365,12 @@
 
 __global__ void alac_classify(alac::DevCfg cfg, const uint8_t* __restrict__ blob, uint64_t blob_bytes, const uint64_t* __restrict__ offsets,
                               const uint32_t* __restrict__ sizes, uint32_t n, uint16_t* __restrict__ keys, uint32_t* __restrict__ sizes_ws,
-                              uint32_t* __restrict__ frames_out, int32_t* __restrict__ status, Plan* plan);
-__global__ void alac_plan(Plan* plan, uint32_t ppw);
+                              Plan* plan, uint32_t ppw);
 __global__ void alac_cu_census(uint32_t* __restrict__ seen, uint32_t* __restrict__ arrived, uint32_t expect);
-__global__ void alac_scatter(const uint16_t* __restrict__ keys, uint32_t n, Plan* plan, uint32_t* __restrict__ perm);
+__global__ void alac_scatter(const uint16_t* __restrict__ keys, uint32_t n, Plan* plan, uint32_t* __restrict__ perm,
+                             uint32_t* __restrict__ frames_out, int32_t* __restrict__ status, uint32_t* __restrict__ other, uint32_t wipe);
 __global__ void alac_task_classify(alac::DevCfg cfg, const alac::ChanDesc* __restrict__ cd, const alac::PktDesc* __restrict__ pd,
-                                   const uint16_t* __restrict__ pkt_keys, uint32_t n_slots, uint16_t* __restrict__ keys, Plan* plan);
+                                   const uint16_t* __restrict__ pkt_keys, uint32_t n_slots, uint16_t* __restrict__ keys, Plan* plan, uint32_t ppw);
 __global__ void alac_scan(alac::DevCfg cfg, const uint8_t* __restrict__ blob, uint64_t blob_bytes, const uint64_t* __restrict__ offsets,
                           const uint32_t* __restrict__ sizes, const uint32_t* __restrict__ perm, const Plan* __restrict__ plan,
                           uint8_t* __restrict__ out, uint64_t out_stride, uint32_t* __restrict__ frames_out,
diff --git a/saprobe-alac_amd/csrc/alacgpu.hip b/saprobe-alac_amd/csrc/alacgpu.hip
--- a/saprobe-alac_amd/csrc/alacgpu.hip
+++ b/saprobe-alac_amd/csrc/alacgpu.hip
@@ -151,10 +151,18 @@
     hipStream_t s_in, s_out;
     hipStream_t s_side;
     hipEvent_t ev_fork, ev_join;
+    hipStream_t s_pre;
+    hipEvent_t ev_pre, ev_scat;
     hipEvent_t ev_start[kTimingSlots], ev_stop[kTimingSlots];
     uint64_t launches;
-    DevBuf scratch_u, scratch_g, plan, cls, perm, sizes_ws;
-    DevBuf cd, pd, plan2, keys2, perm2, rows;
+    DevBuf scratch_u, scratch_g, perm;
+    DevBuf plan[2], cls[2], sizes_ws[2];
+    DevBuf cd, pd, plan2[2], keys2, perm2, rows;
+    size_t plan_used[2], plan2_used[2];
+    uint64_t seq;
+    uint32_t last_half;
+    bool plan_foul;
+    int pre;
     Slot slots[kSlots];
     CopyPool* pool;
     uint32_t n_cu;
@@ -250,26 +258,73 @@
 
 size_t row_stride_of(uint32_t frame_length) { return ((size_t)frame_length + 3u) & ~(size_t)3u; }
 
+struct Grower {
+    alacgpu_decoder* dec;
+    bool quiet = false, zeroed = false;
+    int quiesce() {
+        if (quiet) return ALACGPU_E_OK;
+        HIP_TRY(hipStreamSynchronize(dec->s_pre));
+        HIP_TRY(hipStreamSynchronize(dec->s_side));
+        HIP_TRY(hipStreamSynchronize(dec->stream));
+        quiet = true;
+        return ALACGPU_E_OK;
+    }
+    int grow(DevBuf& b, size_t bytes) {
+        if (bytes <= b.cap) return ALACGPU_E_OK;
+        if (int rc = quiesce()) return rc;
+        return b.ensure(bytes);
+    }
+    int zero(DevBuf& b, size_t& used) {
+        if (b.p) HIP_TRY(hipMemsetAsync(b.p, 0, b.cap, dec->stream));
+        used = 0;
+        zeroed = true;
+        return ALACGPU_E_OK;
+    }
+    int grow_plan(DevBuf& b, size_t& used, size_t bytes) {
+        if (bytes <= b.cap) return ALACGPU_E_OK;
+        if (int rc = grow(b, bytes)) return rc;
+        return zero(b, used);
+    }
+    int settle() {
+        if (zeroed) HIP_TRY(hipStreamSynchronize(dec->stream));
+        zeroed = false;
+        return ALACGPU_E_OK;
+    }
+};
+
 int reserve_workspace(alacgpu_decoder* dec, size_t n, uint32_t ppw) {
     const size_t waves = max_waves(dec, n, ppw);
     int rc;
-    if ((rc = dec->scratch_u.ensure(waves * u_tile_cells(dec->cfg.frame_length) * sizeof(int32_t)))) return rc;
-    if ((rc = dec->scratch_g.ensure(waves * kFallbackSlots * ppw * sizeof(int32_t)))) return rc;
-    if ((rc = dec->plan.ensure(plan_bytes(waves)))) return rc;
-    if ((rc = dec->cls.ensure((n ? n : 1) * sizeof(uint16_t)))) return rc;
-    if ((rc = dec->perm.ensure((n ? n : 1) * sizeof(uint32_t)))) return rc;
-    if ((rc = dec->sizes_ws.ensure((n ? n : 1) * sizeof(uint32_t)))) return rc;
+    Grower g{dec};
+    if (dec->plan_foul) {
+        if ((rc = g.quiesce())) return rc;
+        for (int h = 0; h < 2; h++) {
+            if ((rc = g.zero(dec->plan[h], dec->plan_used[h]))) return rc;
+            if ((rc = g.zero(dec->plan2[h], dec->plan2_used[h]))) return rc;
+        }
+        if ((rc = g.settle())) return rc;
+        dec->plan_foul = false;
+    }
+    if ((rc = g.grow(dec->scratch_u, waves * u_tile_cells(dec->cfg.frame_length) * sizeof(int32_t)))) return rc;
+    if ((rc = g.grow(dec->scratch_g, waves * kFallbackSlots * ppw * sizeof(int32_t)))) return rc;
+    if ((rc = g.grow(dec->perm, (n ? n : 1) * sizeof(uint32_t)))) return rc;
+    for (int h = 0; h < 2; h++) {
+        if ((rc = g.grow_plan(dec->plan[h], dec->plan_used[h], plan_bytes(waves)))) return rc;
+        if ((rc = g.grow(dec->cls[h], (n ? n : 1) * sizeof(uint16_t)))) return rc;
+        if ((rc = g.grow(dec->sizes_ws[h], (n ? n : 1) * sizeof(uint32_t)))) return rc;
+    }
     const size_t ns = (n ? n : 1) * 8;
-    if ((rc = dec->cd.ensure(ns * sizeof(alac::ChanDesc)))) return rc;
-    if ((rc = dec->pd.ensure((n ? n : 1) * sizeof(alac::PktDesc)))) return rc;
+    if ((rc = g.grow(dec->cd, ns * sizeof(alac::ChanDesc)))) return rc;
+    if ((rc = g.grow(dec->pd, (n ? n : 1) * sizeof(alac::PktDesc)))) return rc;
     if (dec->cfg.num_channels > 2) {
-        if ((rc = dec->plan2.ensure(sizeof(Plan)))) return rc;
-        if ((rc = dec->keys2.ensure(ns * sizeof(uint16_t)))) return rc;
-        if ((rc = dec->perm2.ensure(ns * sizeof(uint32_t)))) return rc;
-        if ((rc = dec->rows.ensure((n ? n : 1) * dec->cfg.num_channels * row_stride_of(dec->cfg.frame_length) * sizeof(int32_t))))
+        for (int h = 0; h < 2; h++)
+            if ((rc = g.grow_plan(dec->plan2[h], dec->plan2_used[h], sizeof(Plan)))) return rc;
+        if ((rc = g.grow(dec->keys2, ns * sizeof(uint16_t)))) return rc;
+        if ((rc = g.grow(dec->perm2, ns * sizeof(uint32_t)))) return rc;
+        if ((rc = g.grow(dec->rows, (n ? n : 1) * dec->cfg.num_channels * row_stride_of(dec->cfg.frame_length) * sizeof(int32_t))))
             return rc;
     }
-    return ALACGPU_E_OK;
+    return g.settle();
 }
 
 struct Launch {
@@ -288,8 +343,11 @@
     hipStream_t irr;
     bool forked;
     uint32_t scan_grid;
-    Plan* plan() const { return (Plan*)dec->plan.p; }
-    const uint32_t* sz() const { return (const uint32_t*)dec->sizes_ws.p; }
+    uint32_t half;
+    bool ahead;
+    Plan* plan() const { return (Plan*)dec->plan[half].p; }
+    const uint16_t* cls() const { return (const uint16_t*)dec->cls[half].p; }
+    const uint32_t* sz() const { return (const uint32_t*)dec->sizes_ws[half].p; }
 };
 
 struct SideFork {
@@ -312,15 +370,44 @@
     }
 };
 
-int sort_pass(const Launch& L, const uint32_t* d_sizes) {
+struct PrePass {
+    alacgpu_decoder* dec;
+    bool ahead;
+    bool open = false, done = false;
+    hipStream_t stream() const { return ahead ? dec->s_pre : dec->stream; }
+    int wait() {
+        if (!ahead) return ALACGPU_E_OK;
+        HIP_TRY(hipStreamWaitEvent(dec->s_pre, dec->ev_scat, 0));
+        open = true;
+        return ALACGPU_E_OK;
+    }
+    int join() {
+        if (!ahead) return ALACGPU_E_OK;
+        HIP_TRY(hipEventRecord(dec->ev_pre, dec->s_pre));
+        HIP_TRY(hipStreamWaitEvent(dec->stream, dec->ev_pre, 0));
+        open = false;
+        return ALACGPU_E_OK;
+    }
+    ~PrePass() {
+        if (open) (void)hipStreamSynchronize(dec->s_pre);
+        if (!done) dec->plan_foul = true;
+    }
+};
+
+int sort_pass(const Launch& L, const uint32_t* d_sizes, PrePass& pre) {
     alacgpu_decoder* dec = L.dec;
     const uint32_t nb = (uint32_t)((L.n + 255) / 256);
-    HIP_TRY(hipMemsetAsync(L.plan(), 0, plan_bytes(L.waves), dec->stream));
-    hipLaunchKernelGGL(alac_classify, dim3(nb), dim3(256), 0, dec->stream, L.c, L.d_blob, L.blob_bytes, L.d_offsets, d_sizes,
-                       (uint32_t)L.n, (uint16_t*)dec->cls.p, (uint32_t*)dec->sizes_ws.p, L.d_frames, L.d_status, L.plan());
-    hipLaunchKernelGGL(alac_plan, dim3(1), dim3(kWave), 0, dec->stream, L.plan(), L.ppw);
-    hipLaunchKernelGGL(alac_scatter, dim3(nb), dim3(256), 0, dec->stream, (const uint16_t*)dec->cls.p, (uint32_t)L.n, L.plan(),
-                       (uint32_t*)dec->perm.p);
+    const uint32_t h = L.half, o = h ^ 1u;
+    int rc;
+    if ((rc = pre.wait())) return rc;
+    hipLaunchKernelGGL(alac_classify, dim3(nb), dim3(256), 0, pre.stream(), L.c, L.d_blob, L.blob_bytes, L.d_offsets, d_sizes,
+                       (uint32_t)L.n, (uint16_t*)dec->cls[h].p, (uint32_t*)dec->sizes_ws[h].p, L.plan(), L.ppw);
+    if ((rc = pre.join())) return rc;
+    hipLaunchKernelGGL(alac_scatter, dim3(nb), dim3(256), 0, dec->stream, L.cls(), (uint32_t)L.n, L.plan(), (uint32_t*)dec->perm.p,
+                       L.d_frames, L.d_status, (uint32_t*)dec->plan[o].p, (uint32_t)(dec->plan_used[o] / sizeof(uint32_t)));
+    HIP_TRY(hipEventRecord(dec->ev_scat, dec->stream));
+    dec->plan_used[o] = 0;
+    dec->plan_used[h] = plan_bytes(L.waves);
     return ALACGPU_E_OK;
 }
 
@@ -377,17 +464,18 @@
 
 int split_pipeline(const Launch& L) {
     alacgpu_decoder* dec = L.dec;
-    Plan* plan2 = (Plan*)dec->plan2.p;
+    const uint32_t h = L.half, o = h ^ 1u;
+    Plan* plan2 = (Plan*)dec->plan2[h].p;
     const size_t n_slots = L.n * 8;
     const uint32_t nb2 = (uint32_t)((n_slots + 255) / 256);
     const uint32_t ppw2 = pick_ppw(L.n * dec->cfg.num_channels);
-    HIP_TRY(hipMemsetAsync(plan2, 0, sizeof(Plan), dec->stream));
     hipLaunchKernelGGL(alac_task_classify, dim3(nb2), dim3(256), 0, dec->stream, L.c, (const alac::ChanDesc*)dec->cd.p,
-                       (const alac::PktDesc*)dec->pd.p, (const uint16_t*)dec->cls.p, (uint32_t)n_slots,
-                       (uint16_t*)dec->keys2.p, plan2);
-    hipLaunchKernelGGL(alac_plan, dim3(1), dim3(kWave), 0, dec->stream, plan2, ppw2);
+                       (const alac::PktDesc*)dec->pd.p, L.cls(), (uint32_t)n_slots, (uint16_t*)dec->keys2.p, plan2, ppw2);
     hipLaunchKernelGGL(alac_scatter, dim3(nb2), dim3(256), 0, dec->stream, (const uint16_t*)dec->keys2.p,
-                       (uint32_t)n_slots, plan2, (uint32_t*)dec->perm2.p);
+                       (uint32_t)n_slots, plan2, (uint32_t*)dec->perm2.p, (uint32_t*)nullptr, (int32_t*)nullptr,
+                       (uint32_t*)dec->plan2[o].p, (uint32_t)(dec->plan2_used[o] / sizeof(uint32_t)));
+    dec->plan2_used[o] = 0;
+    dec->plan2_used[h] = sizeof(Plan);
     hipLaunchKernelGGL(alac_chan_predict, dim3((uint32_t)max_waves(16u, n_slots, ppw2)), dim3(kWave), 0, dec->stream, L.c,
                        L.d_blob, L.blob_bytes, L.d_offsets, L.sz(), (const uint32_t*)dec->perm2.p, (const Plan*)plan2,
                        (const alac::ChanDesc*)dec->cd.p, (int32_t*)dec->rows.p, (uint64_t)row_stride_of(dec->cfg.frame_length), ppw2);
@@ -409,7 +497,7 @@
 }
 
 int launch(alacgpu_decoder* dec, const uint8_t* d_blob, uint64_t blob_bytes, const uint64_t* d_offsets,
-           const uint32_t* d_sizes, size_t n, uint8_t* d_out, size_t out_stride, uint32_t* d_frames, int32_t* d_status) {
+           const uint32_t* d_sizes, size_t n, uint8_t* d_out, size_t out_stride, uint32_t* d_frames, int32_t* d_status, bool ahead) {
     if (n == 0) return ALACGPU_E_OK;
     if (n > 0x7fffffffu) {
         set_err("batch too large");
@@ -423,11 +511,13 @@
     dec->last_cap = dec->last_fit5 = 0;
     const Kernels& k = dec->kernels;
     Launch L{dec, dec->dev_cfg, d_blob, blob_bytes, d_offsets, n, d_out, out_stride, d_frames, d_status, ppw, max_waves(dec, n, ppw),
-             dec->stream, false, 0u};
+             dec->stream, false, 0u, (uint32_t)(dec->seq & 1u), ahead && dec->pre != 0};
+    dec->last_half = L.half;
     L.c.aligned16 = (out_stride % 16 == 0 && (reinterpret_cast<uintptr_t>(d_out) % 16) == 0) ? 1u : 0u;
     const uint32_t slot = (uint32_t)(dec->launches % kTimingSlots);
     HIP_TRY(hipEventRecord(dec->ev_start[slot], dec->stream));
-    if ((rc = sort_pass(L, d_sizes))) return rc;
+    PrePass pre{dec, L.ahead};
+    if ((rc = sort_pass(L, d_sizes, pre))) return rc;
     L.forked = k.one_or_two && k.lean &&
                (dec->side >= 2 || (dec->side == 1 && (n + ppw - 1) / ppw <= (size_t)6 * dec->n_cu));
     L.scan_grid = (uint32_t)std::min<size_t>(L.waves, (size_t)(L.forked ? 2u : 6u) * dec->n_cu);
@@ -448,6 +538,8 @@
     if (L.forked && (rc = side.join())) return rc;
     HIP_TRY(hipEventRecord(dec->ev_stop[slot], dec->stream));
     dec->launches++;
+    dec->seq++;
+    pre.done = true;
     return ALACGPU_E_OK;
 }
 
@@ -477,8 +569,9 @@
 }
 
 std::vector<DevBuf*> device_buffers(alacgpu_decoder* d) {
-    std::vector<DevBuf*> v = {&d->scratch_u, &d->scratch_g, &d->plan, &d->cls, &d->perm, &d->sizes_ws, &d->cd, &d->pd,
-                              &d->plan2, &d->keys2, &d->perm2, &d->rows, &d->wave_ws};
+    std::vector<DevBuf*> v = {&d->scratch_u, &d->scratch_g, &d->plan[0], &d->plan[1], &d->cls[0], &d->cls[1], &d->perm,
+                              &d->sizes_ws[0], &d->sizes_ws[1], &d->cd, &d->pd, &d->plan2[0], &d->plan2[1], &d->keys2, &d->perm2,
+                              &d->rows, &d->wave_ws};
     for (Slot& s : d->slots) v.insert(v.end(), {&s.d_in, &s.d_out});
     return v;
 }
@@ -487,13 +580,14 @@
     for (Slot& s : d->slots) v.insert(v.end(), {&s.h_in, &s.h_out});
     return v;
 }
-std::vector<hipStream_t*> streams_of(alacgpu_decoder* d) { return {&d->stream, &d->s_in, &d->s_out, &d->s_side}; }
+std::vector<hipStream_t*> streams_of(alacgpu_decoder* d) { return {&d->stream, &d->s_in, &d->s_out, &d->s_side, &d->s_pre}; }
 struct EventRef {
     hipEvent_t* ev;
     unsigned flags;
 };
 std::vector<EventRef> events_of(alacgpu_decoder* d) {
     std::vector<EventRef> v = {{&d->ev_fork, hipEventDisableTiming}, {&d->ev_join, hipEventDisableTiming},
+                               {&d->ev_pre, hipEventDisableTiming}, {&d->ev_scat, hipEventDisableTiming},
                                {&d->ev_w0, hipEventDefault}, {&d->ev_w1, hipEventDefault},
                                {&d->ev_c0, hipEventDefault}, {&d->ev_c1, hipEventDefault}};
     for (uint32_t i = 0; i < kTimingSlots; i++) v.insert(v.end(), {{&d->ev_start[i], hipEventDefault}, {&d->ev_stop[i], hipEventDefault}});
@@ -543,6 +637,8 @@
     if (const char* e = getenv("ALACGPU_LANES_MIN")) d->lanes_min = (uint32_t)std::max(1, atoi(e));
     d->side = 2;
     if (const char* e = getenv("ALACGPU_SIDE")) d->side = atoi(e);
+    d->pre = 1;
+    if (const char* e = getenv("ALACGPU_PRE")) d->pre = atoi(e);
     d->chunk_bytes = (size_t)192 << 20;
     if (const char* e = getenv("ALACGPU_CHUNK_MB")) {
         const long v = atol(e);
@@ -759,7 +855,7 @@
     int rc = check_decode_args(d, d_blob, blob_bytes, d_offsets, n, d_out, out_stride, d_frames, d_status);
     if (rc) return rc;
     HIP_TRY(hipSetDevice(d->device));
-    rc = launch(d, d_blob, (uint64_t)blob_bytes, d_offsets, d_sizes, n, d_out, out_stride, d_frames, d_status);
+    rc = launch(d, d_blob, (uint64_t)blob_bytes, d_offsets, d_sizes, n, d_out, out_stride, d_frames, d_status, true);
     if (rc) return rc;
     if (sync) HIP_TRY(hipStreamSynchronize(d->stream));
     return ALACGPU_E_OK;
@@ -860,7 +956,7 @@
         uint32_t* d_fr = (uint32_t*)(d_pcm + cnt * d_stride);
         int32_t* d_st = (int32_t*)(d_fr + cnt);
         if ((rc = launch(d, d_in + meta_pad, in_bytes, (const uint64_t*)d_in, (const uint32_t*)(d_in + (cnt + 1) * sizeof(uint64_t)), cnt,
-                         d_pcm, d_stride, d_fr, d_st)))
+                         d_pcm, d_stride, d_fr, d_st, false)))
             return rc;
         HIP_TRY(hipEventRecord(s.ev_k, d->stream));
         HIP_TRY(hipStreamWaitEvent(d->s_out, s.ev_k, 0));
@@ -905,6 +1001,7 @@
         (void)hipStreamSynchronize(d->s_in);
         (void)hipStreamSynchronize(d->stream);
         (void)hipStreamSynchronize(d->s_side);
+        (void)hipStreamSynchronize(d->s_pre);
         (void)hipStreamSynchronize(d->s_out);
         for (int k = 0; k < kSlots; k++) d->slots[k].busy = false;
         return rc;
@@ -970,12 +1067,13 @@
     HIP_TRY(hipSetDevice(d->device));
     HIP_TRY(hipStreamSynchronize(d->stream));
     *n_out = 0;
-    if (!d->plan.p) return ALACGPU_E_OK;
+    const DevBuf& plan = d->plan[d->last_half];
+    if (!plan.p) return ALACGPU_E_OK;
     Plan head;
-    HIP_TRY(hipMemcpy(&head, d->plan.p, sizeof(Plan), hipMemcpyDeviceToHost));
+    HIP_TRY(hipMemcpy(&head, plan.p, sizeof(Plan), hipMemcpyDeviceToHost));
     const size_t n = std::min<size_t>(head.total_waves, max_n / 4);
-    if (plan_bytes(n) > d->plan.cap) return ALACGPU_E_ARG;
-    if (n) HIP_TRY(hipMemcpy(tags, (const uint8_t*)d->plan.p + plan_claims_offset(), n * 4 * sizeof(uint32_t), hipMemcpyDeviceToHost));
+    if (plan_bytes(n) > plan.cap) return ALACGPU_E_ARG;
+    if (n) HIP_TRY(hipMemcpy(tags, (const uint8_t*)plan.p + plan_claims_offset(), n * 4 * sizeof(uint32_t), hipMemcpyDeviceToHost));
     *n_out = n;
     return ALACGPU_E_OK;
 }
@@ -985,9 +1083,10 @@
     HIP_TRY(hipSetDevice(d->device));
     HIP_TRY(hipStreamSynchronize(d->stream));
     memset(out, 0, sizeof(*out));
-    if (!d->plan.p || d->last_n == 0) return ALACGPU_E_OK;
+    const DevBuf& plan = d->plan[d->last_half];
+    if (!plan.p || d->last_n == 0) return ALACGPU_E_OK;
     Plan head;
-    HIP_TRY(hipMemcpy(&head, d->plan.p, sizeof(Plan), hipMemcpyDeviceToHost));
+    HIP_TRY(hipMemcpy(&head, plan.p, sizeof(Plan), hipMemcpyDeviceToHost));
     out->packets_per_slot = d->last_ppw;
     out->slots = head.total_waves;
     out->irregular_slots = head.irr_waves;
diff --git a/saprobe-alac_amd/csrc/k_sort.hip b/saprobe-alac_amd/csrc/k_sort.hip
--- a/saprobe-alac_amd/csrc/k_sort.hip
+++ b/saprobe-alac_amd/csrc/k_sort.hip
@@ -2,49 +2,13 @@
 
 namespace alack {
 
-__global__ void __launch_bounds__(256)
-alac_classify(alac::DevCfg cfg, const uint8_t* __restrict__ blob, uint64_t blob_bytes, const uint64_t* __restrict__ offsets,
-              const uint32_t* __restrict__ sizes, uint32_t n, uint16_t* __restrict__ keys, uint32_t* __restrict__ sizes_ws,
-              uint32_t* __restrict__ frames_out, int32_t* __restrict__ status, Plan* plan) {
-    __shared__ uint32_t hist[kKeys];
-    for (uint32_t k = threadIdx.x; k < kKeys; k += blockDim.x) hist[k] = 0;
+__device__ __forceinline__ void plan_scan(Plan* plan, uint32_t ppw, uint32_t* cnt, uint32_t* wsum) {
+    constexpr uint32_t T = 256, NW = T / kWave;
+    for (uint32_t k = threadIdx.x; k < kKeys; k += T) cnt[k] = __hip_atomic_load(&plan->count[k], __ATOMIC_RELAXED, __HIP_MEMORY_SCOPE_AGENT);
     __syncthreads();
-    const uint32_t i = blockIdx.x * blockDim.x + threadIdx.x;
-    if (i < n) {
-        const uint64_t off = offsets[i];
-        uint64_t sz = sizes ? (uint64_t)sizes[i] : offsets[i + 1] - off;
-        const bool ok = off <= blob_bytes && sz <= blob_bytes - off && sz <= 0x0fffffffull &&
-                        (sizes || offsets[i + 1] >= off);
-        if (!ok) {
-            keys[i] = (uint16_t)alac::TASK_NONE;
-            sizes_ws[i] = 0;
-            frames_out[i] = 0;
-            status[i] = ALACGPU_ERR_RANGE;
-        } else if (sz == 0) {
-            keys[i] = (uint16_t)alac::TASK_NONE;
-            sizes_ws[i] = 0;
-            frames_out[i] = 0;
-            status[i] = ALACGPU_STATUS(alac::ST_OVERRUN, 0, 0);
-        } else {
-            sizes_ws[i] = (uint32_t)sz;
-            const uint8_t* p = blob + off;
-            uint32_t key = alac::classify_regular(cfg, p, (uint32_t)sz, avail_of(blob_bytes, off));
-            if (key == alac::KEY_IRREGULAR) key = alac::lean_config(cfg) ? kKeyScan : kKeyLegacy;
-            keys[i] = (uint16_t)key;
-            atomicAdd(&hist[key], 1u);
-        }
-    }
-    __syncthreads();
-    for (uint32_t k = threadIdx.x; k < kKeys; k += blockDim.x)
-        if (hist[k]) atomicAdd(&plan->count[k], hist[k]);
-}
-
-__global__ void __launch_bounds__(kWave) alac_plan(Plan* plan, uint32_t ppw) {
-    __shared__ uint32_t cnt[kKeys];
-    for (uint32_t k = threadIdx.x; k < kKeys; k += kWave) cnt[k] = plan->count[k];
-    __syncthreads();
-    constexpr uint32_t R = (kKeys + kWave - 1) / kWave;
+    constexpr uint32_t R = (kKeys + T - 1) / T;
     const uint32_t q0 = threadIdx.x * R;
+    const uint32_t lane = threadIdx.x & (kWave - 1u), wave = threadIdx.x / kWave;
     uint32_t p = 0, w = 0, z = 0, wi = 0, ww = 0;
     for (uint32_t r = 0; r < R; ++r) {
         const uint32_t q = q0 + r;
@@ -64,7 +28,7 @@
         const uint32_t tp = (uint32_t)__shfl_up((int)ip, o, kWave), tw = (uint32_t)__shfl_up((int)iw, o, kWave);
         const uint32_t tz = (uint32_t)__shfl_up((int)iz, o, kWave), ti = (uint32_t)__shfl_up((int)ii, o, kWave);
         const uint32_t tx = (uint32_t)__shfl_up((int)ix, o, kWave);
-        if ((int)threadIdx.x >= o) {
+        if ((int)lane >= o) {
             ix += tx;
             ip += tp;
             iw += tw;
@@ -72,6 +36,22 @@
             ii += ti;
         }
     }
+    if (lane == kWave - 1u) {
+        wsum[wave * 5u + 0u] = ip;
+        wsum[wave * 5u + 1u] = iw;
+        wsum[wave * 5u + 2u] = iz;
+        wsum[wave * 5u + 3u] = ii;
+        wsum[wave * 5u + 4u] = ix;
+    }
+    __syncthreads();
+    for (uint32_t v = 0; v < NW; ++v)
+        if (v < wave) {
+            ip += wsum[v * 5u + 0u];
+            iw += wsum[v * 5u + 1u];
+            iz += wsum[v * 5u + 2u];
+            ii += wsum[v * 5u + 3u];
+            ix += wsum[v * 5u + 4u];
+        }
     uint32_t ep = ip - p, ew = iw - w, ez = iz - z;
     for (uint32_t r = 0; r < R; ++r) {
         const uint32_t q = q0 + r;
@@ -88,7 +68,7 @@
             ew += (c + ppw - 1) / ppw;
         }
     }
-    if (threadIdx.x == kWave - 1u) {
+    if (threadIdx.x == T - 1u) {
         plan->nk = iz;
         plan->total_waves = iw;
         plan->irr_waves = ii;
@@ -96,29 +76,85 @@
     }
 }
 
+__device__ __forceinline__ bool plan_by_last_block(Plan* plan, uint32_t ppw, uint32_t* hist, uint32_t* wsum) {
+    __shared__ uint32_t s_last;
+    __threadfence();
+    __syncthreads();
+    if (threadIdx.x == 0) s_last = atomicAdd(&plan->ticket, 1u) == gridDim.x - 1u ? 1u : 0u;
+    __syncthreads();
+    if (!s_last) return false;
+    __threadfence();
+    plan_scan(plan, ppw, hist, wsum);
+    return true;
+}
+
 __global__ void __launch_bounds__(256)
-alac_scatter(const uint16_t* __restrict__ keys, uint32_t n, Plan* plan, uint32_t* __restrict__ perm) {
+alac_classify(alac::DevCfg cfg, const uint8_t* __restrict__ blob, uint64_t blob_bytes, const uint64_t* __restrict__ offsets,
+              const uint32_t* __restrict__ sizes, uint32_t n, uint16_t* __restrict__ keys, uint32_t* __restrict__ sizes_ws,
+              Plan* plan, uint32_t ppw) {
+    __shared__ uint32_t hist[kKeys];
+    __shared__ uint32_t wsum[20];
+    for (uint32_t k = threadIdx.x; k < kKeys; k += blockDim.x) hist[k] = 0;
+    __syncthreads();
+    const uint32_t i = blockIdx.x * blockDim.x + threadIdx.x;
+    if (i < n) {
+        const uint64_t off = offsets[i];
+        uint64_t sz = sizes ? (uint64_t)sizes[i] : offsets[i + 1] - off;
+        const bool ok = off <= blob_bytes && sz <= blob_bytes - off && sz <= 0x0fffffffull &&
+                        (sizes || offsets[i + 1] >= off);
+        if (!ok) {
+            keys[i] = (uint16_t)kKeyRange;
+            sizes_ws[i] = 0;
+        } else if (sz == 0) {
+            keys[i] = (uint16_t)kKeyEmpty;
+            sizes_ws[i] = 0;
+        } else {
+            sizes_ws[i] = (uint32_t)sz;
+            const uint8_t* p = blob + off;
+            uint32_t key = alac::classify_regular(cfg, p, (uint32_t)sz, avail_of(blob_bytes, off));
+            if (key == alac::KEY_IRREGULAR) key = alac::lean_config(cfg) ? kKeyScan : kKeyLegacy;
+            keys[i] = (uint16_t)key;
+            atomicAdd(&hist[key], 1u);
+        }
+    }
+    __syncthreads();
+    for (uint32_t k = threadIdx.x; k < kKeys; k += blockDim.x)
+        if (hist[k]) atomicAdd(&plan->count[k], hist[k]);
+    (void)plan_by_last_block(plan, ppw, hist, wsum);
+}
+
+__global__ void __launch_bounds__(256)
+alac_scatter(const uint16_t* __restrict__ keys, uint32_t n, Plan* plan, uint32_t* __restrict__ perm,
+             uint32_t* __restrict__ frames_out, int32_t* __restrict__ status, uint32_t* __restrict__ other, uint32_t wipe) {
     __shared__ uint32_t hist[kKeys];
     __shared__ uint32_t base[kKeys];
     for (uint32_t k = threadIdx.x; k < kKeys; k += blockDim.x) hist[k] = 0;
     __syncthreads();
     const uint32_t i = blockIdx.x * blockDim.x + threadIdx.x;
     uint32_t key = 0, local = 0;
+    bool sorted = false;
     if (i < n) {
         key = keys[i];
-        if (key != alac::TASK_NONE) local = atomicAdd(&hist[key], 1u);
+        sorted = key < kKeyRange;
+        if (sorted) local = atomicAdd(&hist[key], 1u);
+        else if (status) {
+            frames_out[i] = 0;
+            status[i] = key == kKeyRange ? ALACGPU_ERR_RANGE : ALACGPU_STATUS(alac::ST_OVERRUN, 0, 0);
+        }
     }
+    for (uint32_t k = i; k < wipe; k += gridDim.x * blockDim.x) other[k] = 0u;
     __syncthreads();
     for (uint32_t k = threadIdx.x; k < kKeys; k += blockDim.x)
         if (hist[k]) base[k] = plan->pkt_start[k] + atomicAdd(&plan->cursor[k], hist[k]);
     __syncthreads();
-    if (i < n && key != alac::TASK_NONE) perm[base[key] + local] = i;
+    if (sorted) perm[base[key] + local] = i;
 }
 
 __global__ void __launch_bounds__(256)
 alac_task_classify(alac::DevCfg cfg, const alac::ChanDesc* __restrict__ cd, const alac::PktDesc* __restrict__ pd,
-                   const uint16_t* __restrict__ pkt_keys, uint32_t n_slots, uint16_t* __restrict__ keys, Plan* plan) {
-    __shared__ uint32_t hist[alac::NUM_TASK_KEYS];
+                   const uint16_t* __restrict__ pkt_keys, uint32_t n_slots, uint16_t* __restrict__ keys, Plan* plan, uint32_t ppw) {
+    __shared__ uint32_t hist[kKeys];
+    __shared__ uint32_t wsum[20];
     if (threadIdx.x < alac::NUM_TASK_KEYS) hist[threadIdx.x] = 0;
     __syncthreads();
     const uint32_t t = blockIdx.x * blockDim.x + threadIdx.x;
@@ -137,6 +173,7 @@
     }
     __syncthreads();
     if (threadIdx.x < alac::NUM_TASK_KEYS && hist[threadIdx.x]) atomicAdd(&plan->count[threadIdx.x], hist[threadIdx.x]);
+    (void)plan_by_last_block(plan, ppw, hist, wsum);
 }
 
 __global__ void __launch_bounds__(kWave) alac_cu_census(uint32_t* __restrict__ seen, uint32_t* __restrict__ arrived, uint32_t expect) {
```

Measured after the change: 259,800 Msamples/s. Within noise of the previous version (-0.1%).
